# likojack/ODAM

Hardware: AMD Instinct MI355X
Metric: frames/sec end-to-end (DETR detect + SQ fit), 640x480 ScanNet, 1/2/4/8 GPU (higher is better)
Workload: dtype f32

## Files before the change

### include/odam_detr.h

```cpp
#ifndef ODAM_DETR_H
#define ODAM_DETR_H
#ifdef __cplusplus
extern "C" {
#endif

typedef struct odam_detr odam_detr;

typedef struct {
    int resnet_blocks[4];
    int hidden_dim;
    int nheads;
    int dim_feedforward;
    int enc_layers;
    int dec_layers;
    int num_queries;
    int num_classes1;
    int angle_bins;
    int max_batch;
    int img_h, img_w;
    int dtype;
    int pre_norm;
    int dilation;
    int basic_block;
} odam_detr_cfg;

int odam_detr_create(const odam_detr_cfg* cfg, odam_detr** out);
int odam_detr_destroy(odam_detr* m);

int odam_detr_set_weight(odam_detr* m, const char* name, const float* data, const long long* shape, int ndim);

int odam_detr_finalize(odam_detr* m);

int odam_detr_feature_hw(const odam_detr* m, int* h, int* w);

int odam_detr_forward(odam_detr* m, const float* img, int B, float* logits, float* boxes, float* angle,
                      float* offset, float* size, float* depth, float* obj_features, void* stream);

int odam_detr_forward_masked(odam_detr* m, const float* img, int B, const unsigned char* key_mask, const float* pos,
                             float* logits, float* boxes, float* angle, float* offset, float* size, float* depth,
                             float* obj_features, void* stream);

int odam_detr_forward_aux(odam_detr* m, const float* img, int B, const unsigned char* key_mask, const float* pos,
                          float* logits, float* boxes, float* angle, float* offset, float* size, float* depth,
                          float* obj_features, int frames_per_layer, void* stream);

int odam_detr_debug_read(odam_detr* m, int B, float* layer4_nchw, float* memory, void* stream);

int odam_detr_postprocess(odam_detr* m, const float* logits, const float* boxes, const float* angle,
                          const float* offset, const float* size, const float* depth, int B, const float* K9,
                          float img_w, float img_h, float* rows, void* stream);

int odam_detr_select(const float* rows, int Q, float threshold, int nms_2d, int* keep_idx, int* n_keep);

int odam_detr_select_pack(const float* rows16, int B, int Q, float threshold, int nms_2d, const float* frame_ids,
                          float seq_w, float seq_h, const float* sincos, int n_bins, float* det_block, int* det_count,
                          int* keep_idx, void* stream);

int odam_detr_preprocess_u8(odam_detr* m, const unsigned char* rgb, int B, int h, int w, const float* mean,
                            const float* std_dev, float* out, void* stream);

int odam_detr_profile_enable(odam_detr* m, int on);
int odam_detr_profile_read(odam_detr* m, int* n_launches, double* total_ms, double* total_flops);
int odam_detr_profile_read_attention(odam_detr* m, int* n_launches, double* total_ms, double* total_flops);


int odam_detr_profile_read_stages(odam_detr* m, int n, int* launches, double* ms, double* flops);

int odam_op_conv2d_nhwc(const float* x, const float* w_packed, const float* scale, const float* bias,
                        const float* residual, float* y, int B, int H, int W, int Cin, int Cout, int KH, int KW,
                        int stride, int pad, int Kpad, int relu, int k_order, void* stream);
int odam_op_conv2d_nhwc_bf16(const void* x, const void* w_packed, const float* scale, const float* bias,
                             const void* residual, void* y, int B, int H, int W, int Cin, int Cout, int KH, int KW,
                             int stride, int pad, int Kpad, int relu, int out_f32, int k_order, void* stream);
int odam_op_conv2d_nhwc_ex(const void* x, const void* w_packed, const float* scale, const float* bias, const void* residual,
                           void* y, int B, int H, int W, int Cin, int Cout, int KH, int KW, int stride, int pad, int dil,
                           int Kpad, int relu, int k_order, int dtype, int out_f32, void* stream);
int odam_op_bottleneck_bf16(const void* x, const void* w2, const float* s2, const float* b2, const void* w3, const float* s3,
                            const float* b3, const void* residual, void* y, const void* w1n, const float* s1n, const float* b1n,
                            void* y_next, int B, int H, int W, int P, int stride, int PN, void* stream);
int odam_op_bottleneck_f32(const float* x, const float* w2, const float* s2, const float* b2, const float* w3, const float* s3,
                           const float* b3, const float* residual, float* y, const float* w1n, const float* s1n, const float* b1n,
                           float* y_next, int B, int H, int W, int P, int stride, int PN, void* stream);
long long odam_op_conv_paths(char* buf, int n, int reset);
int odam_op_conv_bf16_mode(int mode);
int odam_op_conv_f32_mode(int mode);
long long odam_op_pooled_stem_launches(void);
int odam_op_attention(const float* Q, int ldq, const float* K, int ldk, const float* V, int ldv, float* O, int ldo,
                      int B, int H, int Lq, int Lk, void* stream);
int odam_op_attention_bf16(const void* Q, int ldq, const void* K, int ldk, const void* V, int ldv, void* O, int ldo,
                           int B, int H, int Lq, int Lk, void* stream);
int odam_op_add_layernorm(const float* x, const float* r, const float* gamma, const float* beta, float* y, int M,
                          void* stream);
int odam_op_attention_ex(const void* Q, int ldq, const void* K, int ldk, const void* V, int ldv, void* O, int ldo,
                         int B, int H, int Lq, int Lk, int head_dim, int dtype, const unsigned char* key_mask, void* stream);
int odam_op_add_layernorm_ex(const void* x, const void* r, const float* gamma, const float* beta, void* y,
                             const float* pos, int L, void* y_pos, int M, int dtype, void* stream);
int odam_op_attention_hd(const void* Q, int ldq, const void* K, int ldk, const void* V, int ldv, void* O, int ldo,
                         int B, int H, int Lq, int Lk, int head_dim, int dtype, const unsigned char* key_mask, void* stream);
int odam_op_add_layernorm_c(const void* x, const void* r, const float* gamma, const float* beta, void* y,
                            const float* pos, int L, void* y_pos, int M, int C, int dtype, void* stream);
int odam_op_quantize_mxfp8(const void* x, int src_dtype, long long n, void* q, void* s, void* stream);
int odam_op_dequantize_mxfp8(const void* q, const void* s, long long n, float* y, void* stream);
int odam_op_conv2d_nhwc_mxfp8(const void* x, const void* xs, const void* w_packed, const void* ws, const float* scale,
                              const float* bias, const void* residual, void* y, void* ys, void* y_bf16, float* y_f32,
                              int B, int H, int W, int Cin, int Cout, int KH, int KW, int stride, int pad, int dil,
                              int Kpad, int relu, int k_order, void* stream);
int odam_op_maxpool3x3s2_nhwc_ex(const void* x, void* y, int B, int H, int W, int C, int dtype, void* stream);
int odam_op_maxpool3x3s2_nhwc(const float* x, float* y, int B, int H, int W, int C, void* stream);
int odam_op_nchw_to_nhwc4(const float* in, void* out, int B, int H, int W, int dtype, int framed, void* stream);
int odam_op_nhwc_to_nchw(const void* in, float* out, int B, int H, int W, int C, int dtype, void* stream);
int odam_op_add_pos(const void* x, const float* pos, int L, void* out, int M, int C, int dtype, void* stream);
int odam_op_to_f32(const void* in, float* out, long long n, int dtype, void* stream);
int odam_op_sigmoid(float* x, int n, void* stream);
int odam_op_postprocess(const float* logits, const float* boxes, const float* angle, const float* offset, const float* size,
                        const float* depth, int n, int n_cls1, int n_bins, const float* K9, float img_w, float img_h, float* rows,
                        void* stream);

#ifdef __cplusplus
}
#endif
#endif
```

### odam_amd/_lib.py

```python
import ctypes
import os

_HERE = os.path.dirname(os.path.abspath(__file__))
LIB_PATH = os.environ.get("ODAM_AMD_LIB") or os.path.join(_HERE, "libodam_amd.so")
_lib = None

c_float_p = ctypes.POINTER(ctypes.c_float)
c_int_p = ctypes.POINTER(ctypes.c_int)
c_void_p = ctypes.c_void_p


class OdamError(RuntimeError):
    pass


_LEGACY_ENV = {"ODAM_CG_BIG": ("cg.ring", False), "ODAM_CG_BIG_F32": ("cg.f32", False), "ODAM_CG_FUSE": ("cg.fuse", False),
               "ODAM_CG_FUSE_BF16": ("cg.fuse_bf16", False), "ODAM_CG_S1": ("cg.s1", False), "ODAM_CG_NO_UT": ("cg.ut", True),
               "ODAM_CG_VARIANT": ("cg.tiles", False), "ODAM_CG_FORCE": ("cg.force", False), "ODAM_CG_NO_PRESPLIT": ("cg.presplit", True),
               "ODAM_ATT_X3": ("att.x3", False), "ODAM_ATT_FP32": ("att.bf16_mfma", True), "ODAM_STEM_ROWS": ("stem.rows", False),
               "ODAM_ASSOC_PERSIST": ("assoc.persist", False), "ODAM_SQ_SPLIT": ("sq.split", False),
               "ODAM_SQ_SPLIT_WAIT": ("sq.split_wait", False), "ODAM_SQ_S": ("sq.lanes", False)}


def _apply_env(L):
    pairs = []
    for name, (key, presence_means_off) in _LEGACY_ENV.items():
        if name in os.environ:
            pairs.append((key, 0 if presence_means_off else int(os.environ[name])))
    for item in filter(None, os.environ.get("ODAM_CONFIG", "").split(",")):
        k, v = item.split("=")
        pairs.append((k.strip(), int(v)))
    for k, v in pairs:
        if L.odam_config_set(k.encode(), ctypes.c_int(v)) != 0:
            raise OdamError(L.odam_last_error().decode("utf-8", "replace"))


def config():
    buf = ctypes.create_string_buffer(1024)
    check(lib().odam_config_describe(buf, 1024), "odam_config_describe")
    return {k: int(v.rstrip("*")) for k, v in (kv.split("=") for kv in buf.value.decode().split())}


def get_config(key):
    v = ctypes.c_int(0)
    check(lib().odam_config_get(key.encode(), ctypes.byref(v)), f"odam_config_get({key})")
    return v.value


def set_config(key, value):
    check(lib().odam_config_set(key.encode(), ctypes.c_int(int(value))), f"odam_config_set({key})")


_I, _P, _F = ctypes.c_int, ctypes.c_void_p, ctypes.c_float
_L, _D = ctypes.c_longlong, ctypes.c_double
_PROTOTYPES = {
    "odam_samples_create": [_I, _I, _L, _L, _P],
    "odam_samples_destroy": [_P],
    "odam_samples_load": [_P, _P, _P, _P, _P, _P, _P, _D, _D, _P],
    "odam_samples_cut": [_P, _I, _P, _P, _P, _I, _P, _P, _P, _P, _I, _P, _P, _P, _P],
    "odam_assoc_ot_batch": [_P, _P, _P, _P, _P, _I, _I, _F, _I, _P, _P, _P, _P, _P, _P, _P],
    "odam_assoc_reserve_batch": [_P, _I, _I],
    "odam_assoc_forward_batch": [_P, _P, _P, _P, _P, _I, _P, _P, _P, _P, _P, _P, _P],
}


def lib():
    global _lib
    if _lib is None:
        if not os.path.exists(LIB_PATH):
            raise OdamError(
                f"{LIB_PATH} not found: build it with `python -c 'import __graft_entry__ as g; g.build()'` "
                "(hipcc --offload-arch=gfx950). There is no CPU fallback.")
        import torch
        L = ctypes.CDLL(LIB_PATH)
        L.odam_last_error.restype = ctypes.c_char_p
        for name, argtypes in _PROTOTYPES.items():
            fn = getattr(L, name)
            fn.argtypes, fn.restype = argtypes, ctypes.c_int
        _apply_env(L)
        _lib = L
    return _lib


def check(code, what):
    if code != 0:
        msg = lib().odam_last_error().decode("utf-8", "replace")
        raise OdamError(f"{what} failed with code {code}: {msg}")


def ptr(t):
    if t is None:
        return c_void_p(0)
    return c_void_p(t.data_ptr())
```

### odam_amd/csrc/cg_args.h

```cpp
#pragma once

namespace odam_cg {

constexpr int ODAM_CG_F32 = 0;
constexpr int ODAM_CG_BF16 = 1;

struct ConvGemmArgs {
    const void* A;
    const void* Wt;
    const void* Wt3 = nullptr;
    const float* scale;
    const float* bias;
    const void* res;
    void* C;
    int B, H, W, Cin, log2Cin;
    int Ho, Wo, Cout;
    int KH, KW, stride, pad;
    int Kpad;
    int relu;
    int M;
    int ldc;
    int dtype;
    int out_f32;
    int lda;
    int k_order;
    const void* F_Wt3 = nullptr;
    const float* F_scale = nullptr;
    const float* F_bias = nullptr;
    const float* F_res = nullptr;
    float* F_C = nullptr;
    int F_ldc = 0, F_relu = 0;
    const void* G_Wt3 = nullptr;
    const float* G_scale = nullptr;
    const float* G_bias = nullptr;
    float* G_C = nullptr;
    int G_N = 64;
    const void* F_Wt = nullptr;
    const void* G_Wt = nullptr;
    int dil = 1;
    int pool = 0, pool_ph = 0, pool_pw = 0, Hp = 0, Wp = 0;
    int no_pin = 0;
    int s1_window = 0;
};

constexpr int POOL_PH = 8, POOL_PW = 14;

}
```

### odam_amd/csrc/cg_big.hpp

```cpp
#pragma once
#include "cg_common.hpp"
#include "cg_tails_f32.hpp"
#include "cg_tail_bf16.hpp"
#include "cg_launch.h"

namespace odam_cg {

constexpr int big_bm(int BN, int NTH) { return (NTH == 1024 && BN == 64) ? 512 : 256; }
constexpr int big_wm(int MODE, int BN, int NTH) {
    return NTH == 1024 ? (BN == 64 ? 16 : 4)
         : MODE >= 3 ? (BN == 256 ? ((MODE == 4 && CG_X16_WM8) ? 8 : 4) : 8) : (BN == 256 ? 2 : (BN == 128 ? 4 : 8));
}
#ifndef CG_DEEP_A
#define CG_DEEP_A 1
#endif

constexpr bool big_deep_a(int MODE, int BN, int NST, int NTH) { return CG_DEEP_A != 0 && MODE == 0 && BN == 256 && NST == 4 && NTH == 1024; }
template <int MODE, int BN, int NST, int NTH>
constexpr int big_lds_bytes() {
    const int bm = big_bm(BN, NTH);
    const int ring = NST * (MODE >= 3 ? bm * 64 + 96 * BN : (bm + BN) * 64);
    const int wm = big_wm(MODE, BN, NTH);
    const int wn = NTH / 64 / wm;
    const int slab = MODE == 4 ? (NTH / 64) * 16 * ((BN / wn > 128 ? 128 : BN / wn) + 4) * 4 : (NTH / 64) * 32 * (BN / wn) * 4;
    const int s1 = (MODE == 0 && NTH == 512) ? (BN == 256 ? 2 : (BN == 128 ? 3 : 4)) * (384 * 64 + 3 * BN * 64) : 0;
    const int m = ring > slab ? ring : slab;
    const int deep = big_deep_a(MODE, BN, NST, NTH) ? (6 + 4) * 256 * 64 : 0;
    const int m2 = m > s1 ? m : s1;
    return m2 > deep ? m2 : deep;
}

template <int MODE, int BN, int NST, int NTH = 512, int FUSE = 0>
__global__ __launch_bounds__(NTH, (NTH == 1024 ? 4 : 2)) void conv_gemm_big_kernel(ConvGemmArgs a) {
    static_assert(!FUSE || (FUSE <= 4 && (MODE == 3 || MODE == 4) && NTH == 512 && ((FUSE != 3 && BN == 64) || (FUSE == 3 && BN == 128))) ||
                      (FUSE >= 5 && FUSE <= 8 && MODE == 0 && NTH == 512 && NST == 4),
                  "fused layers: pre-split filters with 64-column tiles (FUSE 1, 2, 4) or 128-column tiles (FUSE 3); bf16 (FUSE 5 + "
                  "log2(PN / 32), 5 = no chained reduce)");
    static_assert(MODE == 0 || MODE == 2 || MODE == 3 || MODE == 4,
                  "bf16 operands, fp32 split, fp32 split with pre-split filters (3: 32x32x16 matrix instruction, 4: 16x16x32)");
    static_assert(MODE != 4 || FUSE <= 4, "the 16x16x32 schedule: its own epilogue, or the fp32 bottleneck tails");
    constexpr bool BF16 = MODE == 0;
    constexpr bool PRE = MODE == 3 || MODE == 4;
    constexpr bool X16 = MODE == 4;
    static_assert(!PRE || NTH == 512 || (X16 && NTH == 1024), "pre-split filters: eight-wave workgroups, or sixteen waves (16x16x32 loop)");
    static_assert(NTH != 1024 || (FUSE == 0 && ((BN == 64 && (X16 || BF16)) || (BN == 256 && BF16))), "sixteen waves: plain layers (512 x 64: bf16 or the 16x16x32 split loop; 256 x 256: bf16)");
    using T = typename std::conditional<BF16, unsigned short, float>::type;
    constexpr int EPC = BF16 ? 8 : 4;
    constexpr int BM = big_bm(BN, NTH), BKE = 4 * EPC;
    constexpr int KU = 2 * BKE;
    constexpr int NW = NTH / 64;
    constexpr int WM = big_wm(MODE, BN, NTH), WN = NW / WM;
    constexpr int TM = BM / WM / 32, TN = BN / WN / 32;
    constexpr int RPP = NTH / 4;
    constexpr int A_LD = BM / RPP, B_LD = (BN + RPP - 1) / RPP;
    constexpr int ROWB = 64;
    constexpr int A_BYTES = BM * ROWB;
    constexpr int STAGE = PRE ? A_BYTES + 3 * BN * 32 : (BM + BN) * ROWB;
    constexpr int NB3 = 3 * BN / 32;
    constexpr int B3_HI = (NB3 + NW - 1) / NW;
    constexpr int LPT = A_LD + (PRE ? B3_HI : B_LD);
    extern __shared__ __align__(16) float smem[];
    typedef __attribute__((address_space(3))) void* lds_ptr_t;
    const T* __restrict__ Ag = reinterpret_cast<const T*>(a.A);
    const T* __restrict__ Wg = reinterpret_cast<const T*>(a.Wt);

    const int tid = threadIdx.x, lane = tid & 63, wave = tid >> 6;
    const int wm = wave / WN, wn = wave % WN;
    const int tiles_n = (a.Cout + BN - 1) / BN;
    int bid = blockIdx.x;
#if CG_STAMP
    const unsigned long long st_entry = __builtin_readcyclecounter();
#endif
    {
        const int nwg = gridDim.x, xcd = bid & 7, q = nwg >> 3, r = nwg & 7;
        bid = (xcd < r ? xcd * (q + 1) : r * (q + 1) + (xcd - r) * q) + (bid >> 3);
    }
    const int tile_m = bid / tiles_n, tile_n = bid - tile_m * tiles_n;
    const int m0 = tile_m * BM, n0 = tile_n * BN;
    constexpr bool POOLABLE = NTH == 1024 && BN == 64 && FUSE == 0 && (MODE == 4 || MODE == 0);
    constexpr int pl_tw = 2 * POOL_PW + 1, pl_rows = (2 * POOL_PH + 1) * pl_tw;
    static_assert(pl_rows <= 512, "a patch fits a 512-row tile");
    int pl_b = 0, pl_y0 = 0, pl_x0 = 0;
    if constexpr (POOLABLE) {
        if (a.pool) {
            const int txs = (a.Wp + POOL_PW - 1) / POOL_PW, tys = (a.Hp + POOL_PH - 1) / POOL_PH;
            pl_b = bid / (tys * txs);
            const int rem = bid - pl_b * tys * txs, ty = rem / txs, tx = rem - ty * txs;
            pl_y0 = 2 * ty * POOL_PH - 1; pl_x0 = 2 * tx * POOL_PW - 1;
        }
    }
    auto pool_store = [&](const float* S) {
        constexpr int SLD = BN + 4;
        const int py0 = (pl_y0 + 1) >> 1, px0 = (pl_x0 + 1) >> 1;
        constexpr int items = POOL_PH * POOL_PW * (BN / 4);
        for (int it = tid; it < items; it += NTH) {
            const int c4p = it & (BN / 4 - 1), pp = it / (BN / 4), ppy = pp / POOL_PW, ppx = pp - ppy * POOL_PW;
            const int py = py0 + ppy, px = px0 + ppx;
            if (py >= a.Hp || px >= a.Wp) continue;
            const float* w0 = S + ((2 * ppy) * pl_tw + 2 * ppx) * SLD + c4p * 4;
            float4 m4 = *reinterpret_cast<const float4*>(w0);
#pragma unroll
            for (int dy = 0; dy < 3; dy++)
#pragma unroll
                for (int dx = 0; dx < 3; dx++) {
                    if (dy == 0 && dx == 0) continue;
                    const float4 v = *reinterpret_cast<const float4*>(w0 + (dy * pl_tw + dx) * SLD);
                    m4.x = fmaxf(m4.x, v.x); m4.y = fmaxf(m4.y, v.y); m4.z = fmaxf(m4.z, v.z); m4.w = fmaxf(m4.w, v.w);
                }
            const size_t o = (((size_t)pl_b * a.Hp + py) * a.Wp + px) * a.ldc + c4p * 4;
            if constexpr (BF16) {
                const unsigned lo = pack_bf16x2(m4.x, m4.y), hi = pack_bf16x2(m4.z, m4.w);
                *reinterpret_cast<uint2*>(reinterpret_cast<unsigned short*>(a.C) + o) = uint2{lo, hi};
            } else {
                *reinterpret_cast<float4*>(reinterpret_cast<float*>(a.C) + o) = m4;
            }
        }
    };
    auto pool_row_ok = [&](int R) {
        const int dy = R / pl_tw, oy = pl_y0 + dy, ox = pl_x0 + R - dy * pl_tw;
        return R < pl_rows && (unsigned)oy < (unsigned)a.Ho && (unsigned)ox < (unsigned)a.Wo;
    };

    const int c4 = tid & 3, r0 = tid >> 2;
    const int hw = a.Ho * a.Wo;
    const int lda = a.lda > 0 ? a.lda : a.Cin;
    const bool plain = a.KH * a.KW == 1 && a.stride == 1 && a.pad == 0;
    const int ntaps = a.KH * a.KW;
    const int kw_inv = (65536 + a.KW - 1) / a.KW;
    const int nt_inv = (65536 + ntaps - 1) / ntaps;
    const int b0 = (POOLABLE && a.pool) ? pl_b : m0 / hw;
    const int csrc = X16 ? (c4 ^ ((lane >> 4) & 1)) : (c4 ^ ((lane >> 4) & 3));
    const int margin = (a.pad * a.W + a.pad) * lda;
    const unsigned long long pa = (unsigned long long)(Ag + (size_t)b0 * a.H * a.W * lda - margin), pw = (unsigned long long)Wg;
    const u32x4 a_rs4 = u32x4{(unsigned)pa, (unsigned)(pa >> 32) & 0xffffu, OOB_VOFF, 0x00020000u};
    const u32x4 w_rs4 = u32x4{(unsigned)pw, (unsigned)(pw >> 32) & 0xffffu, OOB_VOFF, 0x00020000u};
    unsigned a_voff[A_LD], a_mask[A_LD], w_voff[B_LD];
#pragma unroll
    for (int i = 0; i < A_LD; i++) {
        const int m = m0 + r0 + RPP * i;
        bool ok = m < a.M;
        const int mm = ok ? m : 0;
        int base, iy0 = 0, ix0 = 0;
        if (POOLABLE && a.pool) {
            const int r = r0 + RPP * i, dy = r / pl_tw, oy = pl_y0 + dy, ox = pl_x0 + r - dy * pl_tw;
            ok = r < pl_rows && (unsigned)oy < (unsigned)a.Ho && (unsigned)ox < (unsigned)a.Wo;
            iy0 = (ok ? oy : 0) * a.stride - a.pad; ix0 = (ok ? ox : 0) * a.stride - a.pad;
            base = ((pl_b * a.H + iy0) * a.W + ix0) * lda;
        } else if (plain) {
            base = mm * lda;
        } else {
            const int b = mm / hw, rem = mm - b * hw, oy = rem / a.Wo, ox = rem - oy * a.Wo;
            iy0 = oy * a.stride - a.pad; ix0 = ox * a.stride - a.pad;
            base = ((b * a.H + iy0) * a.W + ix0) * lda;
        }
        a_voff[i] = (unsigned)(base - b0 * a.H * a.W * lda + margin + csrc * EPC) * (unsigned)sizeof(T);
        unsigned mk = plain ? 1u : 0u;
        for (int t = 0; t < (plain ? 0 : ntaps); t++) {
            const int ky = (t * kw_inv) >> 16, kx = t - ky * a.KW;
            if ((unsigned)(iy0 + ky * a.dil) < (unsigned)a.H && (unsigned)(ix0 + kx * a.dil) < (unsigned)a.W) mk |= 1u << t;
        }
        a_mask[i] = ok ? mk : 0u;
    }
#pragma unroll
    for (int i = 0; i < B_LD; i++) {
        const int n = n0 + r0 + RPP * i;
        w_voff[i] = (n < a.Cout && r0 + RPP * i < BN) ? (unsigned)(n * a.Kpad + csrc * EPC) * (unsigned)sizeof(T) : OOB_VOFF;
    }
    const unsigned lds_base = (unsigned)(size_t)(lds_ptr_t)smem;
    const int wave_u = __builtin_amdgcn_readfirstlane(wave);
    const bool b_wave = PRE ? (NB3 % NW == 0 || wave_u < NB3 % NW)
                            : (BN >= RPP || wave_u * 16 < BN);
    unsigned w3_voff[B3_HI > 0 ? B3_HI : 1];
    u32x4 w3_rs4 = w_rs4;
    if constexpr (PRE) {
        const unsigned long long p3 = (unsigned long long)a.Wt3;
        w3_rs4 = u32x4{(unsigned)p3, (unsigned)(p3 >> 32) & 0xffffu, OOB_VOFF, 0x00020000u};
#pragma unroll
        for (int j = 0; j < B3_HI; j++) {
            const int q = wave_u + NW * j;
            const int pl = q / (BN / 32), rb = q - pl * (BN / 32);
            const int row = rb * 32 + (lane >> 1);
            const int n = n0 + row;
            const int cs = X16 ? (lane & 1) : ((lane & 1) ^ ((lane >> 4) & 1));
            w3_voff[j] = (q < NB3 && n < a.Cout) ? (unsigned)(n * (a.Kpad / 16) * 96 + pl * 32 + cs * 16) : OOB_VOFF;
        }
    }

    struct TilePrep { int tap, soff_a, soff_b; };
    auto tile_prep = [&](int kt) {
        int tap, cbase;
        if (a.k_order) {
            const int ku = kt >> 1, chunk = (ku * nt_inv) >> 16;
            tap = ku - chunk * ntaps;
            cbase = chunk * KU + (kt & 1) * BKE;
        } else {
            const int kb = kt * BKE;
            tap = kb >> a.log2Cin;
            cbase = kb & (a.Cin - 1);
        }
        const int ky = (tap * kw_inv) >> 16, kx = tap - ky * a.KW;
        return TilePrep{tap, ((ky * a.W + kx) * a.dil * lda + cbase) * (int)sizeof(T), PRE ? kt * 96 : kt * BKE * (int)sizeof(T)};
    };
    auto dma_part = [&](const TilePrep& tp, int st, int part) {
        const unsigned sb = lds_base + (unsigned)(st * STAGE + wave_u * 16 * ROWB);
        if (part < A_LD) {
            const unsigned vo = ((a_mask[part] >> tp.tap) & 1u) ? a_voff[part] : OOB_VOFF;
            lds_dma16(a_rs4, sb + (unsigned)(RPP * part * ROWB), vo, tp.soff_a);
        } else if constexpr (PRE) {
// ... 86 lines not shown
            for (int j = 0; j < TN; j++) {
                b0[j] = *reinterpret_cast<const float4*>(Bb + j * 32 * ROWB + fq[0]);
                b1[j] = *reinterpret_cast<const float4*>(Bb + j * 32 * ROWB + fq[1]);
            }
            a0 = *reinterpret_cast<const float4*>(Ab + fq[0]);
            a1 = *reinterpret_cast<const float4*>(Ab + fq[1]);
            int part = 0;
            issue_next(part++);
#pragma unroll
            for (; part < LPT; part++) issue_next(part);
#pragma unroll
            for (int j = 0; j < TN; j++) split8(b0[j], b1[j], bh[j], bm[j], bl[j]);
#pragma unroll
            for (int i = 0; i < TM; i++) {
                uint4 ah, am, al;
                split8(a0, a1, ah, am, al);
                if (i + 1 < TM) {
                    a0 = *reinterpret_cast<const float4*>(Ab + (i + 1) * 32 * ROWB + fq[0]);
                    a1 = *reinterpret_cast<const float4*>(Ab + (i + 1) * 32 * ROWB + fq[1]);
                }
#define ODAM_MM(x, y) acc[i][j] = __builtin_amdgcn_mfma_f32_32x32x16_bf16(__builtin_bit_cast(bf16x8, x), __builtin_bit_cast(bf16x8, y), acc[i][j], 0, 0, 0)
#pragma unroll
                for (int j = 0; j < TN; j++) {
                    ODAM_MM(al, bh[j]); ODAM_MM(am, bm[j]); ODAM_MM(ah, bl[j]);
                    ODAM_MM(am, bh[j]); ODAM_MM(ah, bm[j]);
                    ODAM_MM(ah, bh[j]);
                }
#undef ODAM_MM
            }
            return;
        }
        mma_ab(Ab, Bb, issue_next);
    };

    const int nk = a.Kpad / BKE;
    if constexpr (X16) {
        constexpr int MI = BM / WM / 16, NJ = BN / WN / 16;
        static_assert(NJ % 4 == 0, "column tiles in groups of four");
        floatx4 c16[MI][NJ];
#pragma unroll
        for (int i = 0; i < MI; i++)
#pragma unroll
            for (int j = 0; j < NJ; j++) c16[i][j] = floatx4{0.f, 0.f, 0.f, 0.f};
        const int r16 = lane & 15, kq = lane >> 4;
        const int akey = (r16 >> 2) & 1;
        const int a_lane = (kq >> 1) * STAGE + (wm * (BM / WM) + r16) * ROWB;
        const int a_c0 = ((2 * (kq & 1)) ^ akey) << 4, a_c1 = ((2 * (kq & 1) + 1) ^ akey) << 4;
        const int b_lane = (kq >> 1) * STAGE + A_BYTES + (wn * (BN / WN) + r16) * 32 + (kq & 1) * 16;
        auto dma_tile = [&](int kt, int st) {
            if (kt >= nk) return;
            const TilePrep tp = tile_prep(kt);
#pragma unroll
            for (int part = 0; part < A_LD; part++) {
                const unsigned vo = ((a_mask[part] >> tp.tap) & 1u) ? a_voff[part] : OOB_VOFF;
                lds_dma16(a_rs4, lds_base + (unsigned)(st * STAGE + wave_u * 16 * ROWB + RPP * part * ROWB), vo, tp.soff_a);
            }
#pragma unroll
            for (int j = 0; j < B3_HI; j++)
                if (j + 1 < B3_HI || b_wave)
                    lds_dma16(w3_rs4, lds_base + (unsigned)(st * STAGE + A_BYTES + (wave_u + NW * j) * 1024), w3_voff[j], tp.soff_b);
        };
        constexpr int NBLK = MI * NJ;
        constexpr int NDMA = 2 * (A_LD + B3_HI);
        auto dma_part16 = [&](int kt, int st, int part) {
            if (kt >= nk) return;
            const TilePrep tp = tile_prep(kt);
            if (part < A_LD) {
                const unsigned vo = ((a_mask[part] >> tp.tap) & 1u) ? a_voff[part] : OOB_VOFF;
                lds_dma16(a_rs4, lds_base + (unsigned)(st * STAGE + wave_u * 16 * ROWB + RPP * part * ROWB), vo, tp.soff_a);
            } else {
                const int j = part - A_LD;
                if (j + 1 < B3_HI || b_wave)
                    lds_dma16(w3_rs4, lds_base + (unsigned)(st * STAGE + A_BYTES + (wave_u + NW * j) * 1024), w3_voff[j < B3_HI ? j : 0], tp.soff_b);
            }
        };
        dma_tile(0, 0); dma_tile(1, 1);
#if CG_HACK & 3
        const size_t hk_off = ((size_t)m0 * a.ldc + n0) * sizeof(float);
        const __amdgpu_buffer_rsrc_t hk_res = __builtin_amdgcn_make_buffer_rsrc(const_cast<char*>(reinterpret_cast<const char*>(a.res ? a.res : a.C)) + hk_off, 0, a.res ? (int)OOB_VOFF : 0, 0x00020000);
        const __amdgpu_buffer_rsrc_t hk_out = __builtin_amdgcn_make_buffer_rsrc(reinterpret_cast<char*>(a.C) + hk_off, 0, (int)OOB_VOFF, 0x00020000);
        u32x4 hk_l[8] = {};
        constexpr int HK_LPR = (BN / WN) / 4, HK_RPI = 64 / HK_LPR;
        const int hk_row0 = wm * (BM / WM) + lane / HK_LPR;
        const unsigned hk_col = (unsigned)(wn * (BN / WN) + (lane % HK_LPR) * 4) * 4u;
#endif
#define ODAM_MM16(accv, x, y) accv = __builtin_amdgcn_mfma_f32_16x16x32_bf16(__builtin_bit_cast(bf16x8, x), __builtin_bit_cast(bf16x8, y), accv, 0, 0, 0)
#if CG_STAMP
        unsigned long long st_acc[4] = {0, 0, 0, 0}, st_prev = __builtin_readcyclecounter();
        const unsigned long long st_loop0 = st_prev;
#endif
        for (int kp = 0; 2 * kp < nk; ++kp) {
            CG_STAMP_AT(3);
            asm volatile("s_waitcnt vmcnt(0)" ::: "memory");
            CG_STAMP_AT(1);
            __builtin_amdgcn_s_barrier();
            asm volatile("" ::: "memory");
            CG_STAMP_AT(0);
            const int s0 = (2 * kp) & 3;
            const char* Sa = lds_c + s0 * STAGE + a_lane;
            const char* Sb = lds_c + s0 * STAGE + b_lane;
            struct Ops { uint4 h, m, l; };
            constexpr int BD = 2;
            Ops A2[2], B2[BD + 1];
            float4 ar0, ar1;
            auto read_b = [&](int nj, Ops& o) {
                const char* bp = Sb + nj * 16 * 32;
                o.h = *reinterpret_cast<const uint4*>(bp);
                o.m = *reinterpret_cast<const uint4*>(bp + BN * 32);
                o.l = *reinterpret_cast<const uint4*>(bp + 2 * BN * 32);
            };
            auto read_a = [&](int mi) {
                ar0 = *reinterpret_cast<const float4*>(Sa + mi * 16 * ROWB + a_c0);
                ar1 = *reinterpret_cast<const float4*>(Sa + mi * 16 * ROWB + a_c1);
            };
            auto half_split = [](const float4& c, Ops& o, int hf) {
                const float v[4] = {c.x, c.y, c.z, c.w};
                unsigned uh[4], um[4], ul[4];
#pragma unroll
                for (int e = 0; e < 4; e++) {
                    uh[e] = __builtin_bit_cast(unsigned, v[e]);
                    const float r1 = v[e] - __builtin_bit_cast(float, uh[e] & 0xffff0000u);
                    um[e] = __builtin_bit_cast(unsigned, r1);
                    ul[e] = __builtin_bit_cast(unsigned, r1 - __builtin_bit_cast(float, um[e] & 0xffff0000u));
                }
                auto pk = [](unsigned lo_, unsigned hi_) { return __builtin_amdgcn_perm(hi_, lo_, 0x07060302u); };
                if (hf == 0) {
                    o.h.x = pk(uh[0], uh[1]); o.h.y = pk(uh[2], uh[3]); o.m.x = pk(um[0], um[1]); o.m.y = pk(um[2], um[3]);
                    o.l.x = pk(ul[0], ul[1]); o.l.y = pk(ul[2], ul[3]);
                } else {
                    o.h.z = pk(uh[0], uh[1]); o.h.w = pk(uh[2], uh[3]); o.m.z = pk(um[0], um[1]); o.m.w = pk(um[2], um[3]);
                    o.l.z = pk(ul[0], ul[1]); o.l.w = pk(ul[2], ul[3]);
                }
            };
            constexpr bool BREG = CG_X16_BREG != 0;
            constexpr int NG = NJ / 4;
            Ops A4[BREG ? MI : 1], Bg[BREG ? 4 : 1];
            read_a(0);
            if constexpr (BREG) {
#pragma unroll
                for (int j = 0; j < 4; j++) read_b(j, Bg[j]);
                half_split(ar0, A4[0], 0); half_split(ar1, A4[0], 1);
            } else {
#pragma unroll
// ... 532 lines not shown
        return;
    }
    if constexpr (FUSE == 4) {
        fused_chain128(a, acc, smem, lds_base, m0, wave, lane);
        return;
    }
    if constexpr (POOLABLE && MODE == 0) {
        if (a.pool) {
            constexpr int SLD = BN + 4;
            static_assert(BM * SLD * 4 <= big_lds_bytes<MODE, BN, NST, NTH>(), "the pooling slab fits the ring");
            float* S = smem;
            const int half = lane >> 5, l32 = lane & 31;
#pragma unroll
            for (int i = 0; i < TM; i++)
#pragma unroll
                for (int j = 0; j < TN; j++) {
                    const int n = wn * (BN / WN) + j * 32 + l32;
                    const float sc = a.scale ? a.scale[n] : 1.0f, bi = a.bias ? a.bias[n] : 0.0f;
#pragma unroll
                    for (int r = 0; r < 16; r++) {
                        const int R = wm * (BM / WM) + i * 32 + (r & 3) + 8 * (r >> 2) + 4 * half;
                        float v = acc[i][j][r] * sc + bi;
                        v = bf2f(f2bf(v));
                        S[R * SLD + n] = (pool_row_ok(R) && v > 0.f) ? v : 0.f;
                    }
                }
            __syncthreads();
            pool_store(S);
            return;
        }
    }
    if constexpr (FUSE >= 5) {
        fused_bf16<BN, FUSE == 5 ? 0 : (32 << (FUSE - 5)), FUSE == 7 ? 2 : 3>(a, acc, smem, lds_base, m0, wm, wn, wave, lane);
        return;
    }
    static_assert(X16 || (WM * WN * 32 * (BN / WN) * 4 <= big_lds_bytes<MODE, BN, NST, NTH>() && NST * STAGE <= big_lds_bytes<MODE, BN, NST, NTH>()),
                  "ring and epilogue staging fit the dynamic LDS");
    if (ep2) epilogue2<BM, BN, WM, WN, TM, TN, BF16>(a, acc, smem, m0, n0, wm, wn, wave, lane);
    else epilogue<BM, BN, WM, WN, TM, TN, BF16>(a, acc, smem, big_lds_bytes<MODE, BN, NST, NTH>() / 4, m0, n0, wm, wn, wave, lane);
}

template <int MODE, int BN, int NST, int NTH = 512>
static int launch_big(const ConvGemmArgs& a_in, int s1_window, hipStream_t stream) {
    ConvGemmArgs a = a_in;
    a.s1_window = s1_window;
    constexpr int bytes = big_lds_bytes<MODE, BN, NST, NTH>();
    static const bool attr_ok = [] {
        return hipFuncSetAttribute((const void*)conv_gemm_big_kernel<MODE, BN, NST, NTH>, hipFuncAttributeMaxDynamicSharedMemorySize, bytes) == hipSuccess;
    }();
    if (!attr_ok) return odam_fail(2, "conv_gemm: cannot raise the dynamic LDS limit");
    constexpr int bm = big_bm(BN, NTH);
    int tiles = ((a.M + bm - 1) / bm) * ((a.Cout + BN - 1) / BN);
    if (a.pool) {
        if (!(NTH == 1024 && BN == 64 && (MODE == 4 || MODE == 0)) || a.Cout != 64 || a.pool_ph != POOL_PH || a.pool_pw != POOL_PW ||
            a.ldc != a.Cout || a.res)
            return odam_fail(1, "conv_gemm: pooled stem asked for where it does not apply");
        tiles = a.B * ((a.Hp + POOL_PH - 1) / POOL_PH) * ((a.Wp + POOL_PW - 1) / POOL_PW);
    }
    hipLaunchKernelGGL((conv_gemm_big_kernel<MODE, BN, NST, NTH>), dim3(tiles), dim3(NTH), bytes, stream, a);
    ODAM_HIP(hipGetLastError());
    return 0;
}


}
```

### odam_amd/csrc/cg_big_f32.hip

```cpp
#include "cg_big.hpp"

namespace odam_cg {

int launch_big_f32(int mode, int bn, int nth, const ConvGemmArgs& a, hipStream_t stream) {
    if (nth == 1024) {
        if (mode == 4 && bn == 64) return launch_big<4, 64, 4, 1024>(a, 0, stream);
    } else if (bn == 256) {
        if (mode == 4) return launch_big<4, 256, 4>(a, 0, stream);
        if (mode == 3) return launch_big<3, 256, 4>(a, 0, stream);
        if (mode == 2) return launch_big<2, 256, 4>(a, 0, stream);
    } else if (bn == 128) {
        if (mode == 4) return launch_big<4, 128, 4>(a, 0, stream);
        if (mode == 3) return launch_big<3, 128, 4>(a, 0, stream);
        if (mode == 2) return launch_big<2, 128, 4>(a, 0, stream);
    } else if (bn == 64) {
        if (mode == 4) return launch_big<4, 64, 4>(a, 0, stream);
        if (mode == 3) return launch_big<3, 64, 4>(a, 0, stream);
        if (mode == 2) return launch_big<2, 64, 4>(a, 0, stream);
    }
    return odam_fail(1, "conv_gemm: ring kernel (fp32): tile shape not built");
}

}
```

### odam_amd/csrc/cg_choice.h

```cpp
#pragma once
#include "cg_args.h"

namespace odam_cg {

struct Switches {
    int ring, f32, fuse, fuse_bf16, s1, ut, tiles, force, presplit, mfma16, pin, small_x3, stem_pool;
};
Switches current_switches();

enum class Family { Refused, Nothing, Small, RingF32, RingBF16, FusedF32, FusedBF16 };

struct Choice {
    Family family = Family::Nothing;
    bool bf16 = false;
    int bm = 0, bn = 0, waves = 0;
    int stages = 2;
    bool ut = false, x3 = false;
    int mode = 0;
    bool pool = false;
    int chain = 0;
    int s1_window = 0;
    int code = 0;
    const char* message = nullptr;
};

Choice choose(const ConvGemmArgs& a, const Switches& sw);

constexpr int PATH_TOKEN_LEN = 40;
void choice_token(const Choice& c, char* tok);

bool fused_second_ok(const ConvGemmArgs& a, const Switches& sw);
bool fused_bf16_ok(const ConvGemmArgs& a, const Switches& sw);
bool pooled_stem_ok(const ConvGemmArgs& a, const Switches& sw);
bool fused_second_ok(const ConvGemmArgs& a);
bool fused_bf16_ok(const ConvGemmArgs& a);
bool pooled_stem_ok(const ConvGemmArgs& a);
bool presplit_applies(int Cout, int Kpad);

void set_big_mode(int mode);
void set_f32_mode(int mode);
int f32_mode();

}
```

### odam_amd/csrc/cg_choice.hip

```cpp
#include "cg_choice.h"

#include <cstdio>

#include "odam_config.h"

namespace odam_cg {

Switches current_switches() {
    using namespace odam_cfg;
    return {get(CG_RING), get(CG_F32),      get(CG_FUSE),   get(CG_FUSE_BF16), get(CG_S1),       get(CG_UT),    get(CG_TILES),
            get(CG_FORCE), get(CG_PRESPLIT), get(CG_MFMA16), get(CG_PIN),       get(CG_SMALL_X3), get(STEM_POOL)};
}

void set_big_mode(int mode) { odam_cfg::set(odam_cfg::CG_RING, mode); }
void set_f32_mode(int mode) { odam_cfg::set(odam_cfg::CG_F32, mode == 1 ? 0 : mode); }
int f32_mode() {
    const Switches sw = current_switches();
    return sw.ring ? sw.f32 : 0;
}

namespace {

inline bool is_bf16(const ConvGemmArgs& a) { return a.dtype == ODAM_CG_BF16; }

// ... 49 lines not shown
    return c;
}

Choice small_tiles(const ConvGemmArgs& a, const Switches& sw, int bm, int bn, int waves, bool deep = false) {
    Choice c;
    c.family = Family::Small;
    c.bf16 = is_bf16(a);
    c.bm = bm; c.bn = bn; c.waves = waves;
    c.ut = sw.ut != 0 && a.Cin % (c.bf16 ? 64 : 32) == 0 && a.KH * a.KW <= 32 && offsets_fit(a, bm);
    c.x3 = !c.bf16 && c.ut && sw.f32 == 2 && sw.small_x3 != 0;
    c.stages = (c.ut && deep) ? 4 : 2;
    return c;
}

}

bool fused_second_ok(const ConvGemmArgs& a, const Switches& sw) {
    if (!sw.fuse || !sw.ring || sw.f32 != 2 || a.dtype != ODAM_CG_F32) return false;
    if (!a.F_Wt3 || !a.F_C || !a.Wt3) return false;
    const bool l1 = a.Cout == 64 && a.F_ldc == 256, l2 = a.Cout == 128 && a.F_ldc == 512 && !a.G_Wt3;
    if ((!l1 && !l2) || a.dil != 1) return false;
    if (!split_planes_fit(a.Cout, a.Kpad) || !fits31((long)a.Ho * a.Wo * a.F_ldc * 4)) return false;
    if (a.G_Wt3 && (sw.fuse < 2 || !a.G_C || (a.G_N != 64 && a.G_N != 128))) return false;
    return ring_eligible(a, sw, a.Cout);
}

bool fused_bf16_ok(const ConvGemmArgs& a, const Switches& sw) {
    if (!sw.fuse_bf16 || !sw.ring || a.dtype != ODAM_CG_BF16 || !a.F_Wt || !a.F_C) return false;
    if (a.Cout != 64 && a.Cout != 128 && a.Cout != 256) return false;
    if (a.F_ldc != 4 * a.Cout || a.KH * a.KW != 9 || a.Cin != a.Cout || !a.k_order || a.dil != 1) return false;
    if (!fits31((long)a.M * a.F_ldc * 2)) return false;
    if (a.G_Wt) {
        if (sw.fuse_bf16 < 2 || !a.G_C) return false;
        const bool built = (a.Cout == 64 && (a.G_N == 64 || a.G_N == 128)) || (a.Cout == 128 && a.G_N == 128);
        if (!built) return false;
    }
    return ring_eligible(a, sw, a.Cout);
}

bool pooled_stem_ok(const ConvGemmArgs& a, const Switches& sw) {
    if (!sw.ring || !(sw.tiles & 8) || sw.stem_pool == 0) return false;
    if (is_bf16(a)) {
        if (!(a.lda > 0 && a.lda < a.Cin) && sw.ring < 2) return false;
        if (is_3x3_stride1(a) || a.out_f32) return false;
    } else if (ring_mode_f32(a, sw) != 4) {
        return false;
    }
    if (a.Cout != 64 || a.ldc != 64 || a.res || !a.relu) return false;
    if (a.pool_ph != POOL_PH || a.pool_pw != POOL_PW) return false;
    if (a.Hp != (a.Ho + 2 - 3) / 2 + 1 || a.Wp != (a.Wo + 2 - 3) / 2 + 1) return false;
    return ring_eligible(a, sw, 64) && fills_512_row_tiles(a, sw);
}

bool fused_second_ok(const ConvGemmArgs& a) { return fused_second_ok(a, current_switches()); }
bool fused_bf16_ok(const ConvGemmArgs& a) { return fused_bf16_ok(a, current_switches()); }
bool pooled_stem_ok(const ConvGemmArgs& a) { return pooled_stem_ok(a, current_switches()); }
bool presplit_applies(int Cout, int Kpad) { return f32_mode() == 2 && split_planes_fit(Cout, Kpad); }

Choice choose(const ConvGemmArgs& a, const Switches& sw) {
    const bool bf = is_bf16(a);
    const int epc = bf ? 8 : 4, taps = a.KH * a.KW;
    if (a.Kpad % (8 * epc) != 0 || a.Cin < epc || (a.Cin & (a.Cin - 1)) != 0 || a.KW > 7 || taps > 64)
        return refuse("conv_gemm: unsupported shape (Kpad % k-tile, Cin a power of two >= one 16-byte chunk, KW <= 7)");
    if (a.k_order && (a.Cin % (8 * epc) != 0 || taps > 32 || a.Kpad / (8 * epc) >= 2048))
        return refuse("conv_gemm: k_order 1 needs Cin % k-tile == 0, at most 32 taps, fewer than 2048 k-tiles");
    if (a.M <= 0 || a.Cout <= 0) return Choice{};

    if (a.pool) {
        if (!pooled_stem_ok(a, sw)) return refuse("conv_gemm: pooled stem asked for where it does not apply (check pooled_stem_ok)");
        return ring(a, sw, bf ? 0 : 4, 64, 16);
    }
    if (a.F_Wt3) {
        if (!fused_second_ok(a, sw)) return refuse("conv_gemm: fused second layer asked for where it does not apply (check fused_second_ok)");
        Choice c;
        c.family = Family::FusedF32;
        c.bm = 256; c.bn = a.Cout; c.waves = 8; c.chain = a.G_Wt3 ? a.G_N : 0;
        c.mode = (a.Kpad % 32 == 0 && (sw.mfma16 >= 3 || (sw.mfma16 == 2 && a.Cout == 128))) ? 4 : 3;
        return c;
    }
    if (a.F_Wt) {
        if (!fused_bf16_ok(a, sw)) return refuse("conv_gemm: fused bf16 bottleneck asked for where it does not apply (check fused_bf16_ok)");
        Choice c;
        c.family = Family::FusedBF16;
        c.bf16 = true;
        c.bm = 256; c.bn = a.Cout; c.waves = 8; c.chain = a.G_Wt ? a.G_N : 0;
        c.s1_window = sw.s1;
        return c;
    }

    if (sw.ring) {
        const bool x3 = !bf && sw.f32 == 2;
        const int mode = bf ? 0 : ring_mode_f32(a, sw);
        if (a.Cout % 256 == 0 || a.Cout >= 384) {
            if (ring_eligible(a, sw, 256))
                return ring(a, sw, mode, 256, (bf && (sw.tiles & 16) && !is_3x3_stride1(a)) ? 16 : 8);
            if (mode >= 3 && ring_eligible(a, sw, 128)) return ring(a, sw, mode, 128, 8);
        } else if (a.Cout > 64 && (sw.ring >= 2 || x3) && ring_eligible(a, sw, 128)) {
            return ring(a, sw, mode, 128, 8);
        } else if (x3 && a.Cout > 32 && a.Cout <= 64 && ring_eligible(a, sw, 64)) {
            return ring(a, sw, mode, 64, (mode == 4 && (sw.tiles & 8) && fills_512_row_tiles(a, sw)) ? 16 : 8);
        } else if (bf && (sw.ring >= 2 || (a.lda > 0 && a.lda < a.Cin)) && a.Cout > 32 && a.Cout <= 64 && ring_eligible(a, sw, 64)) {
            return ring(a, sw, mode, 64, ((sw.tiles & 8) && !is_3x3_stride1(a) && fills_512_row_tiles(a, sw)) ? 16 : 8);
        }
    }

    if (sw.force == 1) return small_tiles(a, sw, 128, 64, 8);
    if (sw.force == 2) return small_tiles(a, sw, 64, 64, 4, true);
    if (sw.force == 3) return small_tiles(a, sw, 128, 128, 4);
    if (a.Cout <= 64) return small_tiles(a, sw, 128, 64, (sw.tiles & 2) ? 8 : 4);
    const long tiles128 = (long)((a.M + 127) / 128) * ((a.Cout + 127) / 128);
    if (tiles128 < 128) return small_tiles(a, sw, 64, 64, 4, (sw.tiles & 4) != 0);
    return small_tiles(a, sw, 128, 128, (sw.tiles & 1) ? 8 : 4);
}

void choice_token(const Choice& c, char* tok) {
    const int n = PATH_TOKEN_LEN;
    tok[0] = 0;
    switch (c.family) {
    case Family::Small:
        std::snprintf(tok, n, "%s.small.%dx%d.w%d%s%s%s", c.bf16 ? "bf16" : "f32", c.bm, c.bn, c.waves, c.ut ? ".ut" : "", c.x3 ? ".x3" : "",
// ... 18 lines not shown
```

### odam_amd/csrc/detr_forward.hip

```cpp
#include <hip/hip_runtime.h>

#include <atomic>

#include "detr_kernels.h"
#include "detr_model.h"
#include "odam_config.h"

using namespace odam_dm;
using odam_cg::ConvGemmArgs;

namespace odam_dm {

ConvGemmArgs conv_args(const Conv& c, const void* x, int B, int H, int W, int dtype) {
    ConvGemmArgs a{};
    a.dtype = dtype;
    a.A = x; a.Wt = c.w; a.Wt3 = c.w3; a.scale = c.scale; a.bias = c.bias;
    a.B = B; a.H = H; a.W = W; a.Cin = c.Cin; a.log2Cin = ilog2(c.Cin);
    a.Ho = conv_out(H, (c.KH - 1) * c.dil + 1, c.stride, c.pad); a.Wo = conv_out(W, (c.KW - 1) * c.dil + 1, c.stride, c.pad);
    a.Cout = c.Cout; a.KH = c.KH; a.KW = c.KW; a.stride = c.stride; a.pad = c.pad; a.Kpad = c.Kpad; a.dil = c.dil;
    a.k_order = c.k_order;
    a.M = B * a.Ho * a.Wo; a.ldc = c.Cout;
    return a;
}

// ... 27 lines not shown
    const int Ho = conv_out(H, (c.KH - 1) * c.dil + 1, c.stride, c.pad), Wo = conv_out(W, (c.KW - 1) * c.dil + 1, c.stride, c.pad);
    const int Cin_true = (c.KH == 7) ? 3 : c.Cin;
    return m->conv_ev.timed(st, 2.0 * B * Ho * Wo * (double)c.Cout * c.KH * c.KW * Cin_true,
                            [&] { return run_conv(c, x, B, H, W, res, relu, y, st, m->dt, out_f32); });
}
int lin_t(odam_detr* m, const Conv& c, const void* x, int M, const void* res, bool relu, void* y, hipStream_t st,
          int out_f32 = 0) {
    return conv_t(m, c, x, 1, 1, M, res, relu, y, st, out_f32);
}

int fused_c2c3_t(odam_detr* m, const Conv& c2, const Conv& c3, const void* x, int B, int H, int W, const void* res, void* y,
                 hipStream_t st, const Conv* next_c1, void* t_next, bool* chained) {
    *chained = false;
    if (m->basic) return -1;
    if (c2.dil != 1) return -1;
    if (c3.KH != 1 || c3.stride != 1 || c3.Kpad != c2.Cout) return -1;
    if (!m->dt && (!c2.w3 || !c3.w3)) return -1;
    ConvGemmArgs a = conv_args(c2, x, B, H, W, m->dt);
    a.relu = 1;
    a.F_scale = c3.scale; a.F_bias = c3.bias; a.F_res = (const float*)res; a.F_C = (float*)y;
    a.F_ldc = c3.Cout; a.F_relu = 1;
    const bool bf = m->dt != 0;
    auto fused_ok = [&] { return bf ? odam_cg::fused_bf16_ok(a) : odam_cg::fused_second_ok(a); };
    if (bf) a.F_Wt = c3.w; else a.F_Wt3 = c3.w3;
    const bool next_ok = next_c1 && t_next && next_c1->KH == 1 && next_c1->stride == 1 && next_c1->Kpad == c3.Cout &&
                         (bf || (next_c1->w3 && (next_c1->Cout == 64 || next_c1->Cout == 128) && c3.Cout == 256));
    if (next_ok) {
        if (bf) a.G_Wt = next_c1->w; else a.G_Wt3 = next_c1->w3;
        a.G_scale = next_c1->scale; a.G_bias = next_c1->bias; a.G_C = (float*)t_next; a.G_N = next_c1->Cout;
        *chained = fused_ok();
        if (!*chained) { a.G_Wt = a.G_Wt3 = nullptr; a.G_scale = a.G_bias = nullptr; a.G_C = nullptr; a.G_N = 64; }
    }
    if (!fused_ok()) return -1;
    const double flops3 = *chained ? 2.0 * a.M * (double)next_c1->Cout * c3.Cout : 0.0;
    return m->conv_ev.timed(st, 2.0 * a.M * ((double)c2.Cout * c2.KH * c2.KW * c2.Cin + (double)c3.Cout * c2.Cout) + flops3,
                            [&] { return odam_cg::launch_conv_gemm(a, st); });
}

std::atomic<long long> g_pooled_stem_launches{0};

int stem_rows_t(odam_detr* m, int B, hipStream_t st, void* pooled_out, bool* pooled) {
    const Conv& c = m->stem_rows;
    ConvGemmArgs a = conv_args(c, m->x4, B, m->cfg.img_h + 6, m->cfg.img_w + 8, m->dt);
    a.lda = 4; a.Ho = m->H1; a.Wo = m->W1; a.M = B * a.Ho * a.Wo;
    a.relu = 1;
    a.pool = 1; a.pool_ph = odam_cg::POOL_PH; a.pool_pw = odam_cg::POOL_PW; a.Hp = m->H2; a.Wp = m->W2; a.C = pooled_out;
    *pooled = odam_cg::pooled_stem_ok(a);
    if (!*pooled) { a.pool = 0; a.C = m->stem_out; }
    else g_pooled_stem_launches.fetch_add(1);
    return m->conv_ev.timed(st, 2.0 * a.M * (double)c.Cout * 147,
                            [&] { return odam_cg::launch_conv_gemm(a, st); });
}

int mx_t(odam_detr* m, const Conv& c, const unsigned char* x, const unsigned char* xs, int B, int H, int W, const void* res, bool relu,
         unsigned char* y, unsigned char* ys, void* yb, hipStream_t st) {
    odam_mx::ConvArgs a = mx_args(c, x, xs, B, H, W);
    a.res = (const unsigned short*)res; a.relu = relu ? 1 : 0;
    a.y = y; a.ys = ys; a.yb = (unsigned short*)yb;
    return m->conv_ev.timed(st, 2.0 * a.M * (double)c.Cout * c.Kpad, [&] { return odam_mx::launch_conv(a, st); });
}

int att_t(odam_detr* m, const void* Q, int ldq, const void* K, int ldk, const void* V, int ldv, void* O, int ldo,
          int B, int H, int Lq, int Lk, hipStream_t st, const unsigned char* key_mask = nullptr) {
    const int hd = m->cfg.hidden_dim / m->cfg.nheads;
    return m->att_ev.timed(st, 4.0 * B * H * (double)Lq * Lk * hd,
                           [&] { return odam_dk::launch_attention(Q, ldq, K, ldk, V, ldv, O, ldo, B, H, Lq, Lk, m->dt, st, key_mask, hd); });
}


struct Act { char *cur, *nxt; int H, W; };

char* off(const odam_detr* m, char* p, size_t n) { return p + n * m->es; }

void mark_stage(odam_detr* m, size_t i) {
    for (int l = 0, first = 0; l < 4; first += m->cfg.resnet_blocks[l], l++)
        if ((int)i == first) m->stage_ev[l + 1] = m->conv_ev.used;
}

int stem(odam_detr* m, const float* img, int B, hipStream_t st) {
    const int dt = m->dt, ih = m->cfg.img_h, iw = m->cfg.img_w;
    const bool rows_ok = odam_cfg::get(odam_cfg::STEM_ROWS) != 0;
    bool pooled = false;
    const long Mst = (long)B * m->H1 * m->W1;
    const bool rows_mode = dt ? (m->stem_rows.w != nullptr && odam_cfg::get(odam_cfg::CG_RING) != 0)
                              : (m->stem_rows.w3 != nullptr && odam_cg::f32_mode() == 2);
    if (rows_ok && rows_mode && (Mst >= 192L * 256 || odam_cfg::get(odam_cfg::CG_PIN))) {
        RC(odam_dk::launch_nchw_to_nhwc4_framed(img, m->x4, B, ih, iw, dt, st));
        RC(stem_rows_t(m, B, st, m->bufA, &pooled));
    } else {
        RC(odam_dk::launch_nchw_to_nhwc4(img, m->x4, B, ih, iw, dt, st));
        RC(conv_t(m, m->stem, m->x4, B, ih, iw, nullptr, true, m->stem_out, st));
    }
    if (!pooled) RC(odam_dk::launch_maxpool3x3s2(m->stem_out, m->bufA, B, m->H1, m->W1, 64, m->H2, m->W2, dt, st));
    return 0;
}

int body_mxfp8(odam_detr* m, int B, Act& s, hipStream_t st) {
    unsigned char *cq = m->qa, *cs = m->qas, *nq = m->qb, *ns = m->qbs;
    RC(odam_mx::launch_quantize(s.cur, 1, (size_t)B * s.H * s.W * 64, cq, cs, st));
    for (size_t i = 0; i < m->blocks.size(); i++) {
        mark_stage(m, i);
        const Bottleneck& b = m->blocks[i];
        const int stride = m->block_stride[i];
        const int Ho = conv_out(s.H, 3, stride, 1), Wo = conv_out(s.W, 3, stride, 1);
        const bool last = i + 1 == m->blocks.size();
        unsigned char* oq = last ? nullptr : nq;
        unsigned char* os = last ? nullptr : ns;
        RC(mx_t(m, b.c1, cq, cs, B, s.H, s.W, nullptr, true, m->qt1, m->qt1s, nullptr, st));
        const char* res = s.cur;
        if (b.has_ds) {
            RC(mx_t(m, b.ds, cq, cs, B, s.H, s.W, nullptr, false, nullptr, nullptr, m->dsb, st));
            res = m->dsb;
        }
        if (m->basic) {
            RC(mx_t(m, b.c2, m->qt1, m->qt1s, B, Ho, Wo, res, true, oq, os, s.nxt, st));
        } else {
            RC(mx_t(m, b.c2, m->qt1, m->qt1s, B, s.H, s.W, nullptr, true, m->qt2, m->qt2s, nullptr, st));
            RC(mx_t(m, b.c3, m->qt2, m->qt2s, B, Ho, Wo, res, true, oq, os, s.nxt, st));
        }
        std::swap(s.cur, s.nxt); std::swap(cq, nq); std::swap(cs, ns);
        s.H = Ho; s.W = Wo;
    }
    return 0;
}

int body_basic(odam_detr* m, int B, Act& s, hipStream_t st) {
    for (size_t i = 0; i < m->blocks.size(); i++) {
        mark_stage(m, i);
        const Bottleneck& b = m->blocks[i];
        const int stride = m->block_stride[i];
        const int Ho = conv_out(s.H, 3, stride, 1), Wo = conv_out(s.W, 3, stride, 1);
        RC(conv_t(m, b.c1, s.cur, B, s.H, s.W, nullptr, true, m->t1, st));
        const char* res = s.cur;
        if (b.has_ds) {
            RC(conv_t(m, b.ds, s.cur, B, s.H, s.W, nullptr, false, m->dsb, st));
            res = m->dsb;
        }
        RC(conv_t(m, b.c2, m->t1, B, Ho, Wo, res, true, s.nxt, st));
        std::swap(s.cur, s.nxt);
        s.H = Ho; s.W = Wo;
    }
    return 0;
}

int body_bottleneck(odam_detr* m, int B, Act& s, hipStream_t st) {
    char* tin = m->t1;
    char* tout = m->t2;
    bool have_c1 = false;
// ... 71 lines not shown
        RC(lin_t(m, m->mlp[k][2], m->h2, Mq, nullptr, false, outs[k], st, 1));
    }
    return odam_dk::launch_sigmoid(boxes, Mq * 4, st);
}

struct LayerOut { float *logits, *boxes, *angle, *offset, *size, *depth, *obj_features; int fpl; };

int layer_heads(odam_detr* m, int B, const LayerOut& o, size_t l, hipStream_t st) {
    const size_t row = l * (size_t)o.fpl * m->cfg.num_queries;
    return heads(m, B, o.logits + row * m->cfg.num_classes1, o.boxes + row * 4, o.angle + row * m->cfg.angle_bins, o.offset + row * 2,
                 o.size + row * 3, o.depth + row, o.obj_features ? o.obj_features + row * m->cfg.hidden_dim : nullptr, st);
}

int decoder(odam_detr* m, int B, const unsigned char* key_mask, hipStream_t st, const LayerOut* each = nullptr) {
    const int E = m->cfg.hidden_dim, Hh = m->cfg.nheads, Q = m->cfg.num_queries, dt = m->dt, L = m->L, Mq = B * Q;
    ODAM_HIP(hipMemsetAsync(m->tgt, 0, (size_t)m->es * Mq * E, st));
    RC(odam_dk::launch_add_pos(nullptr, m->query_pos, Q, m->tgtpos, Mq, dt, st, E));
    const int ldkv = m->cfg.dec_layers * E;
    for (size_t i = 0; i < m->dec.size(); i++) {
        const DecLayer& d = m->dec[i];
        if (m->cfg.pre_norm) {
            RC(odam_dk::launch_add_layernorm(m->tgt, nullptr, d.n1.g, d.n1.b, m->dtmp, m->query_pos, Q, m->tgtpos, Mq, dt, st, E));
            RC(lin_t(m, d.qk, m->tgtpos, Mq, nullptr, false, m->dqk, st));
            RC(lin_t(m, d.v, m->dtmp, Mq, nullptr, false, m->dv, st));
            RC(att_t(m, m->dqk, 2 * E, off(m, m->dqk, E), 2 * E, m->dv, E, m->datt, E, B, Hh, Q, Q, st));
            RC(lin_t(m, d.out, m->datt, Mq, m->tgt, false, m->tgt, st));
            RC(odam_dk::launch_add_layernorm(m->tgt, nullptr, d.n2.g, d.n2.b, m->dtmp, m->query_pos, Q, m->tgtpos, Mq, dt, st, E));
            RC(lin_t(m, d.cq, m->tgtpos, Mq, nullptr, false, m->dq, st));
            RC(att_t(m, m->dq, E, off(m, m->kc, i * E), ldkv, off(m, m->vc, i * E), ldkv, m->datt, E, B, Hh, Q, L, st, key_mask));
            RC(lin_t(m, d.cout, m->datt, Mq, m->tgt, false, m->tgt, st));
            RC(odam_dk::launch_add_layernorm(m->tgt, nullptr, d.n3.g, d.n3.b, m->dtmp, nullptr, Q, nullptr, Mq, dt, st, E));
            RC(lin_t(m, d.l1, m->dtmp, Mq, nullptr, true, m->dffn, st));
            RC(lin_t(m, d.l2, m->dffn, Mq, m->tgt, false, m->tgt, st));
            if (each) RC(layer_heads(m, B, *each, i, st));
            continue;
        }
        RC(lin_t(m, d.qk, m->tgtpos, Mq, nullptr, false, m->dqk, st));
        RC(lin_t(m, d.v, m->tgt, Mq, nullptr, false, m->dv, st));
        RC(att_t(m, m->dqk, 2 * E, off(m, m->dqk, E), 2 * E, m->dv, E, m->datt, E, B, Hh, Q, Q, st));
        RC(lin_t(m, d.out, m->datt, Mq, m->tgt, false, m->dtmp, st));
        RC(odam_dk::launch_add_layernorm(m->dtmp, nullptr, d.n1.g, d.n1.b, m->tgt, m->query_pos, Q, m->tgtpos, Mq, dt, st, E));
        RC(lin_t(m, d.cq, m->tgtpos, Mq, nullptr, false, m->dq, st));
        RC(att_t(m, m->dq, E, off(m, m->kc, i * E), ldkv, off(m, m->vc, i * E), ldkv, m->datt, E, B, Hh, Q, L, st, key_mask));
        RC(lin_t(m, d.cout, m->datt, Mq, m->tgt, false, m->dtmp, st));
        RC(odam_dk::launch_add_layernorm(m->dtmp, nullptr, d.n2.g, d.n2.b, m->tgt, nullptr, Q, nullptr, Mq, dt, st, E));
        RC(lin_t(m, d.l1, m->tgt, Mq, nullptr, true, m->dffn, st));
        RC(lin_t(m, d.l2, m->dffn, Mq, m->tgt, false, m->dtmp, st));
        RC(odam_dk::launch_add_layernorm(m->dtmp, nullptr, d.n3.g, d.n3.b, m->tgt, m->query_pos, Q, m->tgtpos, Mq, dt, st, E));
        if (each) RC(layer_heads(m, B, *each, i, st));
    }
    return 0;
}

int forward_impl(odam_detr* m, const float* img, int B, const unsigned char* key_mask, const float* pos_b,
                 float* logits, float* boxes, float* angle, float* offset, float* size, float* depth,
                 float* obj_features, void* stream, int frames_per_layer = 0) {
    if (!m || !img || !logits || !boxes || !angle || !offset || !size || !depth)
        return odam_fail(1, "odam_detr_forward: null pointer");
    if (!m->finalized) return odam_fail(1, "odam_detr_forward: call odam_detr_finalize first");
    if (B < 1 || B > m->cfg.max_batch) return odam_fail(3, "odam_detr_forward: batch outside 1..max_batch");
    hipStream_t st = (hipStream_t)stream;
    m->conv_ev.used = m->att_ev.used = 0;

    RC(stem(m, img, B, st));
    std::fill(m->stage_ev, m->stage_ev + 6, m->conv_ev.used);
    m->stage_ev[0] = 0;
    Act s{m->bufA, m->bufB, m->H2, m->W2};
    RC(m->mx ? body_mxfp8(m, B, s, st) : m->basic ? body_basic(m, B, s, st) : body_bottleneck(m, B, s, st));
    m->layer4 = s.cur;
    m->stage_ev[5] = m->conv_ev.used;

    const int E = m->cfg.hidden_dim, M = B * m->L;
    RC(conv_t(m, m->input_proj, s.cur, B, s.H, s.W, nullptr, false, m->src, st));
    const float* pos = pos_b ? pos_b : m->pos;
    const int Lp = pos_b ? M : m->L;
    RC(odam_dk::launch_add_pos(m->src, pos, Lp, m->srcpos, M, m->dt, st, E));
    RC(encoder(m, B, pos, Lp, key_mask, st));
    RC(lin_t(m, m->cross_k_all, m->srcpos, M, nullptr, false, m->kc, st));
    RC(lin_t(m, m->cross_v_all, m->memory_out, M, nullptr, false, m->vc, st));

    if (frames_per_layer > 0) {
        const LayerOut each{logits, boxes, angle, offset, size, depth, obj_features, frames_per_layer};
        return decoder(m, B, key_mask, st, &each);
    }
    RC(decoder(m, B, key_mask, st));
    return heads(m, B, logits, boxes, angle, offset, size, depth, obj_features, st);
}

}

extern "C" int odam_detr_forward(odam_detr* m, const float* img, int B, float* logits, float* boxes, float* angle,
                                 float* offset, float* size, float* depth, float* obj_features, void* stream) {
    return forward_impl(m, img, B, nullptr, nullptr, logits, boxes, angle, offset, size, depth, obj_features, stream);
}

extern "C" int odam_detr_forward_masked(odam_detr* m, const float* img, int B, const unsigned char* key_mask,
                                        const float* pos, float* logits, float* boxes, float* angle, float* offset,
                                        float* size, float* depth, float* obj_features, void* stream) {
    if (!key_mask || !pos) return odam_fail(1, "odam_detr_forward_masked: null mask / position table");
    return forward_impl(m, img, B, key_mask, pos, logits, boxes, angle, offset, size, depth, obj_features, stream);
}

extern "C" int odam_detr_forward_aux(odam_detr* m, const float* img, int B, const unsigned char* key_mask, const float* pos,
                                     float* logits, float* boxes, float* angle, float* offset, float* size, float* depth,
                                     float* obj_features, int frames_per_layer, void* stream) {
    if (!m || !img || !logits || !boxes || !angle || !offset || !size || !depth) return odam_fail(1, "odam_detr_forward_aux: null pointer");
    if ((key_mask == nullptr) != (pos == nullptr))
        return odam_fail(1, "odam_detr_forward_aux: mask and position table go together (both null for a same-size batch)");
    if (frames_per_layer < 1 || frames_per_layer < B) return odam_fail(1, "odam_detr_forward_aux: frames_per_layer below the batch");
    if (!m->finalized) return odam_fail(1, "odam_detr_forward_aux: call odam_detr_finalize first");
    return forward_impl(m, img, B, key_mask, pos, logits, boxes, angle, offset, size, depth, obj_features, stream, frames_per_layer);
}

extern "C" int odam_detr_debug_read(odam_detr* m, int B, float* layer4_nchw, float* memory, void* stream) {
    if (!m || !m->finalized || !m->layer4) return odam_fail(1, "odam_detr_debug_read: no forward has run");
    hipStream_t st = (hipStream_t)stream;
    if (layer4_nchw) RC(odam_dk::launch_nhwc_to_nchw(m->layer4, layer4_nchw, B, m->fh, m->fw, m->l4_ch, m->dt, st));
    if (memory) RC(odam_dk::launch_to_f32(m->memory_out ? m->memory_out : m->src, memory, (size_t)B * m->L * m->cfg.hidden_dim, m->dt, st));
    return 0;
}

extern "C" int odam_detr_postprocess(odam_detr* m, const float* logits, const float* boxes, const float* angle,
                                     const float* offset, const float* size, const float* depth, int B,
                                     const float* K9, float img_w, float img_h, float* rows, void* stream) {
    if (!m || !logits || !boxes || !angle || !offset || !size || !depth || !K9 || !rows)
        return odam_fail(1, "odam_detr_postprocess: null pointer");
    return odam_dk::launch_postprocess(logits, boxes, angle, offset, size, depth, B, m->cfg.num_queries,
                                       m->cfg.num_classes1, m->cfg.angle_bins, img_w, img_h, K9[0], K9[4], K9[2],
                                       K9[5], rows, (hipStream_t)stream);
}

extern "C" long long odam_op_pooled_stem_launches(void) { return g_pooled_stem_launches.load(); }

extern "C" int odam_detr_profile_enable(odam_detr* m, int on) {
    if (!m) return odam_fail(1, "odam_detr_profile_enable: null model");
    m->conv_ev.on = m->att_ev.on = on != 0;
    m->conv_ev.used = m->att_ev.used = 0;
    return 0;
}

extern "C" int odam_detr_profile_read(odam_detr* m, int* n_launches, double* total_ms, double* total_flops) {
    if (!m || !n_launches || !total_ms || !total_flops) return odam_fail(1, "odam_detr_profile_read: null argument");
    return m->conv_ev.sum(0, m->conv_ev.used, n_launches, total_ms, total_flops);
}

extern "C" int odam_detr_profile_read_stages(odam_detr* m, int n, int* launches, double* ms, double* flops) {
// ... 11 lines not shown
```

### odam_amd/csrc/detr_input.hip

```cpp
#include <hip/hip_runtime.h>

#include <cmath>

#include "detr_kernels.h"
#include "detr_model.h"

using namespace odam_dm;

static int resample_table(odam_detr* m, int in_size, int out_size, odam_detr::Resample* r) {
    auto it = m->resample.find({in_size, out_size});
    if (it != m->resample.end()) { *r = it->second; return 0; }
    const double scale = (double)in_size / out_size;
    const double filterscale = scale < 1.0 ? 1.0 : scale;
    const double support = 1.0 * filterscale;
    const int ksize = (int)std::ceil(support) * 2 + 1;
    std::vector<int> xmin(out_size), cnt(out_size), K((size_t)out_size * ksize, 0);
    std::vector<double> w(ksize);
    const double ss = 1.0 / filterscale;
    for (int xx = 0; xx < out_size; xx++) {
        const double center = (xx + 0.5) * scale;
        int lo = (int)(center - support + 0.5);
        if (lo < 0) lo = 0;
        int hi = (int)(center + support + 0.5);
        if (hi > in_size) hi = in_size;
        const int n = hi - lo;
        double ww = 0.0;
        for (int x = 0; x < ksize; x++) w[x] = 0.0;
        for (int x = 0; x < n; x++) {
            double t = (x + lo - center + 0.5) * ss;
            if (t < 0.0) t = -t;
            w[x] = t < 1.0 ? 1.0 - t : 0.0;
            ww += w[x];
        }
        for (int x = 0; x < n; x++)
            if (ww != 0.0) w[x] /= ww;
        for (int x = 0; x < ksize; x++)
            K[(size_t)xx * ksize + x] = w[x] < 0 ? (int)(-0.5 + w[x] * (1 << 22)) : (int)(0.5 + w[x] * (1 << 22));
        xmin[xx] = lo; cnt[xx] = n;
    }
    odam_detr::Resample t{};
    t.ksize = ksize;
    if (int rc = m->dev_alloc(&t.xmin, xmin.size())) return rc;
    if (int rc = m->dev_alloc(&t.cnt, cnt.size())) return rc;
    if (int rc = m->dev_alloc(&t.K, K.size())) return rc;
    ODAM_HIP(hipMemcpy(t.xmin, xmin.data(), xmin.size() * sizeof(int), hipMemcpyHostToDevice));
    ODAM_HIP(hipMemcpy(t.cnt, cnt.data(), cnt.size() * sizeof(int), hipMemcpyHostToDevice));
    ODAM_HIP(hipMemcpy(t.K, K.data(), K.size() * sizeof(int), hipMemcpyHostToDevice));
    m->resample[{in_size, out_size}] = t;
    *r = t;
    return 0;
}

extern "C" int odam_detr_preprocess_u8(odam_detr* m, const unsigned char* rgb, int B, int h, int w, const float* mean,
                                       const float* stdv, float* out, void* stream) {
    if (!m || !rgb || !mean || !stdv || !out) return odam_fail(1, "odam_detr_preprocess_u8: null pointer");
    if (B < 0 || h < 1 || w < 1) return odam_fail(1, "odam_detr_preprocess_u8: bad size");
    odam_detr::Resample tx{}, ty{};
    RC(resample_table(m, w, m->cfg.img_w, &tx));
    RC(resample_table(m, h, m->cfg.img_h, &ty));
    return odam_dk::launch_preprocess_u8(rgb, B, h, w, tx.xmin, tx.cnt, tx.K, tx.ksize, ty.xmin, ty.cnt, ty.K, ty.ksize,
                                         out, m->cfg.img_h, m->cfg.img_w, mean, stdv, (hipStream_t)stream);
}

extern "C" int odam_detr_select(const float* rows, int Q, float threshold, int nms_2d, int* keep_idx, int* n_keep) {
    if (!rows || !keep_idx || !n_keep || Q < 0) return odam_fail(1, "odam_detr_select: bad argument");
    std::vector<int> cand;
    for (int q = 0; q < Q; q++)
        if (rows[(size_t)q * 16] > threshold) cand.push_back(q);
    std::stable_sort(cand.begin(), cand.end(), [&](int a, int b) { return rows[(size_t)a * 16] < rows[(size_t)b * 16]; });
    std::reverse(cand.begin(), cand.end());
    const int n = (int)cand.size();
    std::vector<char> sup(n, 0);
    auto box3 = [&](int q, float lo[3], float hi[3]) {
        const float* r = rows + (size_t)q * 16;
        for (int k = 0; k < 3; k++) {
            lo[k] = (-r[10 + k]) / 2.0f + r[6 + k];
            hi[k] = r[10 + k] / 2.0f + r[6 + k];
        }
    };
    int nk = 0;
    for (int i = 0; i < n; i++) {
        if (sup[i]) continue;
        const int s = cand[i];
        keep_idx[nk++] = s;
        float slo[3], shi[3];
        box3(s, slo, shi);
        const float* rs = rows + (size_t)s * 16;
        for (int j = i + 1; j < n; j++) {
            if (sup[j]) continue;
            const int t = cand[j];
            const float* rt = rows + (size_t)t * 16;
            float tlo[3], thi[3];
            box3(t, tlo, thi);
            float inter = 1.0f, va = 1.0f, vb = 1.0f;
            {
                const float dx = std::max(0.0f, std::min(shi[0], thi[0]) - std::max(slo[0], tlo[0]));
                const float dy = std::max(0.0f, std::min(shi[1], thi[1]) - std::max(slo[1], tlo[1]));
                const float dz = std::max(0.0f, std::min(shi[2], thi[2]) - std::max(slo[2], tlo[2]));
                inter = dx * dy * dz;
                va = (shi[0] - slo[0]) * (shi[1] - slo[1]) * (shi[2] - slo[2]);
                vb = (thi[0] - tlo[0]) * (thi[1] - tlo[1]) * (thi[2] - tlo[2]);
            }
            const float iou3 = inter / (va + vb - inter);
// ... 15 lines not shown
```

### odam_amd/csrc/detr_kernels.h

```cpp
#pragma once
#include <hip/hip_runtime.h>

namespace odam_dk {

int launch_attention(const void* Q, int ldq, const void* K, int ldk, const void* V, int ldv, void* O, int ldo,
                     int B, int H, int Lq, int Lk, int dtype, hipStream_t stream, const unsigned char* key_mask = nullptr,
                     int head_dim = 32);

int launch_attention_d64(const float* Q, int ldq, const float* K, int ldk, const float* V, int ldv, float* O, int ldo,
                         int B, int H, int Lq, int Lk, hipStream_t stream);

int launch_add_layernorm(const void* x, const void* r, const float* gamma, const float* beta, void* y,
                         const float* pos, int L, void* y_pos, int M, int dtype, hipStream_t stream, int C = 256);

int launch_add_pos(const void* x, const float* pos, int L, void* out, int M, int dtype, hipStream_t stream, int C = 256);

int launch_nchw_to_nhwc4(const float* in, void* out, int B, int H, int W, int dtype, hipStream_t stream);
int launch_nchw_to_nhwc4_framed(const float* in, void* out, int B, int H, int W, int dtype, hipStream_t stream);

int launch_maxpool3x3s2(const void* in, void* out, int B, int H, int W, int C, int Ho, int Wo, int dtype,
                        hipStream_t stream);

int launch_nhwc_to_nchw(const void* in, float* out, int B, int H, int W, int C, int dtype, hipStream_t stream);

int launch_to_f32(const void* in, float* out, size_t n, int dtype, hipStream_t stream);

int launch_sigmoid(float* x, int n, hipStream_t stream);

int launch_postprocess(const float* logits, const float* boxes, const float* angle, const float* offset,
                       const float* size, const float* depth, int B, int Q, int n_cls1, int n_bins, float img_w,
                       float img_h, float fx, float fy, float cx, float cy, float* rows, hipStream_t stream);

int launch_preprocess_u8(const unsigned char* rgb, int B, int h, int w, const int* tx_xmin, const int* tx_cnt,
                         const int* tx_K, int tx_ksize, const int* ty_xmin, const int* ty_cnt, const int* ty_K,
                         int ty_ksize, float* out, int H, int W, const float mean[3], const float stdv[3],
                         hipStream_t stream);

}
```

### odam_amd/csrc/detr_kernels.hip

```cpp
#include "detr_kernels.h"

#include <cstdlib>

#include "odam_config.h"
#include "odam_err.h"

namespace odam_dk {

typedef float floatx16 __attribute__((ext_vector_type(16)));
typedef unsigned short bf16_t;

__device__ __forceinline__ float bf2f(bf16_t u) { return __builtin_bit_cast(float, (unsigned)u << 16); }
__device__ __forceinline__ bf16_t f2bf(float f) { return __builtin_bit_cast(bf16_t, (__bf16)f); }
__device__ __forceinline__ unsigned pack_bf16x2(float lo, float hi) {
    typedef float f32x2_t __attribute__((ext_vector_type(2)));
    typedef __bf16 bf16x2_t __attribute__((ext_vector_type(2)));
    return __builtin_bit_cast(unsigned, __builtin_convertvector(f32x2_t{lo, hi}, bf16x2_t));
}
__device__ __forceinline__ float4 ld4(const float* p) { return *reinterpret_cast<const float4*>(p); }
__device__ __forceinline__ float4 ld4(const bf16_t* p) {
    const ushort4 u = *reinterpret_cast<const ushort4*>(p);
    return float4{bf2f(u.x), bf2f(u.y), bf2f(u.z), bf2f(u.w)};
}
__device__ __forceinline__ void st4(float* p, float4 v) { *reinterpret_cast<float4*>(p) = v; }
__device__ __forceinline__ void st4(bf16_t* p, float4 v) {
    *reinterpret_cast<uint2*>(p) = uint2{pack_bf16x2(v.x, v.y), pack_bf16x2(v.z, v.w)};
}
#define ODAM_DISPATCH(dtype, KERNEL, ...)                                                  \
    do {                                                                                  \
        if ((dtype) == 1) { KERNEL(bf16_t, __VA_ARGS__); } else { KERNEL(float, __VA_ARGS__); } \
    } while (0)

constexpr int ATT_KT = 32;

__device__ __forceinline__ int acc_row(int r, int half) { return (r & 3) + 8 * (r >> 2) + 4 * half; }

template <typename T, int D>
__global__ __launch_bounds__(256) void attention_kernel(const T* __restrict__ Q, int ldq,
                                                        const T* __restrict__ K, int ldk,
                                                        const T* __restrict__ V, int ldv,
                                                        T* __restrict__ O, int ldo, int Lq, int Lk, float scale,
                                                        const unsigned char* __restrict__ key_mask) {
    constexpr int LD = D + 4;
    constexpr int HD = D / 2;
    constexpr int NO = D / 32;
    constexpr int CPR = D / 4;
    constexpr int RPP = 256 / CPR;
    __shared__ __align__(16) float Ks[2][ATT_KT][LD];
    __shared__ __align__(16) float Vs[2][ATT_KT][LD];

    const int tid = threadIdx.x, lane = tid & 63, wave = tid >> 6;
    const int half = lane >> 5, col = lane & 31;
    const int h = blockIdx.y, b = blockIdx.z;
    const int q0 = blockIdx.x * 128 + wave * 32;
    const T* Qb = Q + (size_t)b * Lq * ldq + h * D;
    const T* Kb = K + (size_t)b * Lk * ldk + h * D;
    const T* Vb = V + (size_t)b * Lk * ldv + h * D;

// ... 827 lines not shown
    float den = 0.0f;
    for (int c = 0; c < n_cls1; c++) den += expf(lg[c] - mx);
    float best = -1.0f;
    int cls = 0;
    for (int c = 0; c < n_cls1 - 1; c++) {
        const float p = expf(lg[c] - mx) / den;
        if (p > best) { best = p; cls = c; }
    }
    const float* bx = boxes + (size_t)i * 4;
    const float x0 = (bx[0] - 0.5f * bx[2]) * img_w, y0 = (bx[1] - 0.5f * bx[3]) * img_h;
    const float x1 = (bx[0] + 0.5f * bx[2]) * img_w, y1 = (bx[1] + 0.5f * bx[3]) * img_h;
    const float d = depth[i];
    const float scx = offset[(size_t)i * 2 + 0] * img_w + (x0 + x1) / 2.0f;
    const float scy = offset[(size_t)i * 2 + 1] * img_h + (y0 + y1) / 2.0f;
    const float c3x = ((scx - cx) / fx) * d;
    const float c3y = ((scy - cy) / fy) * d;
    const float* an = angle + (size_t)i * n_bins;
    int ab = 0;
    float am = an[0];
    for (int k = 1; k < n_bins; k++)
        if (an[k] > am) { am = an[k]; ab = k; }
    float* o = rows + (size_t)i * 16;
    o[0] = best; o[1] = (float)cls;
    o[2] = x0; o[3] = y0; o[4] = x1; o[5] = y1;
    o[6] = c3x; o[7] = c3y; o[8] = d;
    o[9] = (float)ab;
    o[10] = size[(size_t)i * 3 + 0]; o[11] = size[(size_t)i * 3 + 1]; o[12] = size[(size_t)i * 3 + 2];
    o[13] = 0.0f; o[14] = 0.0f; o[15] = 0.0f;
}

int launch_postprocess(const float* logits, const float* boxes, const float* angle, const float* offset,
                       const float* size, const float* depth, int B, int Q, int n_cls1, int n_bins, float img_w,
                       float img_h, float fx, float fy, float cx, float cy, float* rows, hipStream_t stream) {
    const int n = B * Q;
    if (n <= 0) return 0;
    hipLaunchKernelGGL(postprocess_kernel, dim3((n + 63) / 64), dim3(64), 0, stream, logits, boxes, angle, offset,
                       size, depth, n, n_cls1, n_bins, img_w, img_h, fx, fy, cx, cy, rows);
    ODAM_HIP(hipGetLastError());
    return 0;
}

struct ResampleTable {
    const int* xmin;
    const int* cnt;
    const int* K;
    int ksize;
};

__device__ __forceinline__ int clip8_22(int v) {
    v >>= 22;
    return v < 0 ? 0 : (v > 255 ? 255 : v);
}

__global__ __launch_bounds__(256) void preprocess_u8_kernel(const unsigned char* __restrict__ rgb, int h, int w,
                                                            ResampleTable tx, ResampleTable ty, int need_x, int need_y,
                                                            float* __restrict__ out, int H, int W, float3 mean,
                                                            float3 stdv) {
    const int X = blockIdx.x * 256 + threadIdx.x;
    const int Y = blockIdx.y;
    const size_t b = blockIdx.z;
    if (X >= W) return;
    const unsigned char* img = rgb + b * (size_t)h * w * 3;
    const int x0 = need_x ? tx.xmin[X] : X, nx = need_x ? tx.cnt[X] : 1;
    const int y0 = need_y ? ty.xmin[Y] : Y, ny = need_y ? ty.cnt[Y] : 1;
    const int* kx = tx.K + (size_t)X * tx.ksize;
    const int* ky = ty.K + (size_t)Y * ty.ksize;
    int acc[3] = {1 << 21, 1 << 21, 1 << 21};
    int last[3] = {0, 0, 0};
    for (int j = 0; j < ny; j++) {
        const unsigned char* row = img + ((size_t)(y0 + j) * w + x0) * 3;
        int hv[3];
        if (need_x) {
            int a0 = 1 << 21, a1 = 1 << 21, a2 = 1 << 21;
            for (int k = 0; k < nx; k++) {
                const int kk = kx[k];
                a0 += row[k * 3 + 0] * kk; a1 += row[k * 3 + 1] * kk; a2 += row[k * 3 + 2] * kk;
            }
            hv[0] = clip8_22(a0); hv[1] = clip8_22(a1); hv[2] = clip8_22(a2);
        } else {
            hv[0] = row[0]; hv[1] = row[1]; hv[2] = row[2];
        }
        if (need_y) {
            const int kk = ky[j];
            acc[0] += hv[0] * kk; acc[1] += hv[1] * kk; acc[2] += hv[2] * kk;
        }
        last[0] = hv[0]; last[1] = hv[1]; last[2] = hv[2];
    }
    const int u0 = need_y ? clip8_22(acc[0]) : last[0];
    const int u1 = need_y ? clip8_22(acc[1]) : last[1];
    const int u2 = need_y ? clip8_22(acc[2]) : last[2];
    const size_t plane = (size_t)H * W, o = (b * 3 * H + Y) * (size_t)W + X;
    out[o] = ((float)u0 / 255.0f - mean.x) / stdv.x;
    out[o + plane] = ((float)u1 / 255.0f - mean.y) / stdv.y;
    out[o + 2 * plane] = ((float)u2 / 255.0f - mean.z) / stdv.z;
}

int launch_preprocess_u8(const unsigned char* rgb, int B, int h, int w, const int* tx_xmin, const int* tx_cnt,
                         const int* tx_K, int tx_ksize, const int* ty_xmin, const int* ty_cnt, const int* ty_K,
                         int ty_ksize, float* out, int H, int W, const float mean[3], const float stdv[3],
                         hipStream_t stream) {
    if (B <= 0) return 0;
    ResampleTable tx{tx_xmin, tx_cnt, tx_K, tx_ksize}, ty{ty_xmin, ty_cnt, ty_K, ty_ksize};
    hipLaunchKernelGGL(preprocess_u8_kernel, dim3((W + 255) / 256, H, B), dim3(256), 0, stream, rgb, h, w, tx, ty,
                       (int)(W != w), (int)(H != h), out, H, W, float3{mean[0], mean[1], mean[2]},
                       float3{stdv[0], stdv[1], stdv[2]});
    ODAM_HIP(hipGetLastError());
    return 0;
}

}
```

### odam_amd/csrc/detr_model.h

```cpp
#pragma once
#include <hip/hip_runtime.h>

#include <algorithm>
#include <map>
#include <string>
#include <utility>
#include <vector>

#include "../../include/odam_detr.h"
#include "cg_mx8.h"
#include "conv_gemm.h"
#include "odam_err.h"

namespace odam_dm {

struct HostTensor {
    std::vector<long long> shape;
    std::vector<float> data;
};

struct Conv {
    void* w = nullptr;
    void* w3 = nullptr;
    float* scale = nullptr;
// ... 53 lines not shown
        }
        return 0;
    }
};

}

struct odam_detr {
    odam_detr_cfg cfg;
    std::map<std::string, odam_dm::HostTensor> host;
    bool finalized = false;
    std::vector<void*> allocs;

    odam_dm::Conv stem;
    bool basic = false;
    int l4_ch = 2048;
    std::vector<odam_dm::Bottleneck> blocks;
    std::vector<int> block_stride;
    odam_dm::Conv input_proj;
    std::vector<odam_dm::EncLayer> enc;
    std::vector<odam_dm::DecLayer> dec;
    odam_dm::Conv cross_k_all, cross_v_all;
    odam_dm::LN dec_norm;
    odam_dm::LN enc_norm;
    const void* memory_out = nullptr;
    odam_dm::Conv class_embed;
    odam_dm::Conv mlp[5][3];
    odam_dm::Conv stem_rows;
    float* pos = nullptr;
    float* query_pos = nullptr;

    int H1, W1, H2, W2, fh, fw, L;

    char *x4 = nullptr, *stem_out = nullptr, *bufA = nullptr, *bufB = nullptr, *t1 = nullptr, *t2 = nullptr,
         *dsb = nullptr;
    char *src = nullptr, *srcpos = nullptr, *qk = nullptr, *v = nullptr, *att = nullptr, *tmp = nullptr, *ffn = nullptr;
    char *kc = nullptr, *vc = nullptr;
    char *tgt = nullptr, *tgtpos = nullptr, *dqk = nullptr, *dv = nullptr, *datt = nullptr, *dq = nullptr,
         *dtmp = nullptr, *dffn = nullptr, *hs = nullptr, *h1 = nullptr, *h2 = nullptr;
    const char* layer4 = nullptr;
    int es = 4;
    int dt = 0;
    bool mx = false;
    unsigned char *qa = nullptr, *qas = nullptr, *qb = nullptr, *qbs = nullptr, *qt1 = nullptr, *qt1s = nullptr, *qt2 = nullptr,
                  *qt2s = nullptr;

    odam_dm::EventLog conv_ev;
    odam_dm::EventLog att_ev;
    size_t stage_ev[6] = {};

    struct Resample { int* xmin; int* cnt; int* K; int ksize; };
    std::map<std::pair<int, int>, Resample> resample;

    template <typename T>
    int dev_alloc(T** p, size_t n) {
        ODAM_HIP(hipMalloc((void**)p, n * sizeof(T)));
        allocs.push_back((void*)*p);
        return 0;
    }
};

namespace odam_dm {

#define RC(call)                 \
    do {                         \
        int rc_ = (call);        \
        if (rc_) return rc_;     \
    } while (0)

odam_cg::ConvGemmArgs conv_args(const Conv& c, const void* x, int B, int H, int W, int dtype);
odam_mx::ConvArgs mx_args(const Conv& c, const void* x, const void* xs, int B, int H, int W);

int run_conv(const Conv& c, const void* x, int B, int H, int W, const void* res, bool relu, void* y, hipStream_t st,
             int dtype = 0, int out_f32 = 0);

}
```

### odam_amd/csrc/detr_ops.hip

```cpp
#include <hip/hip_runtime.h>

#include "detr_kernels.h"
#include "detr_model.h"

using namespace odam_dm;
using odam_cg::ConvGemmArgs;

namespace {

int fail(int code, const char* who, const char* what) {
    std::snprintf(g_odam_err, sizeof(g_odam_err), "%s: %s", who, what);
    return code;
}

int split_filters_for_call(const float* w_packed, int Cout, int Kpad, hipStream_t st, unsigned short** d3, const char* who) {
    *d3 = nullptr;
    if (!odam_cg::presplit_applies(Cout, Kpad)) return 0;
    std::vector<float> hw((size_t)Cout * Kpad);
    ODAM_HIP(hipStreamSynchronize(st));
    ODAM_HIP(hipMemcpy(hw.data(), w_packed, hw.size() * sizeof(float), hipMemcpyDeviceToHost));
    std::vector<unsigned short> h3(hw.size() * 3);
    odam_cg::split3_filters(hw.data(), Cout, Kpad, h3.data());
    ODAM_HIP(hipMalloc(d3, h3.size() * 2));
    if (hipMemcpy(*d3, h3.data(), h3.size() * 2, hipMemcpyHostToDevice) != hipSuccess) {
// ... 124 lines not shown
extern "C" int odam_op_conv2d_nhwc_mxfp8(const void* x, const void* xs, const void* w_packed, const void* ws, const float* scale,
                                         const float* bias, const void* residual, void* y, void* ys, void* y_bf16, float* y_f32,
                                         int B, int H, int W, int Cin, int Cout, int KH, int KW, int stride, int pad, int dil,
                                         int Kpad, int relu, int k_order, void* stream) {
    if (dil != 1) return odam_fail(1, "odam_op_conv2d_nhwc_mxfp8: dilation must be 1");
    if (k_order != 0) return odam_fail(1, "odam_op_conv2d_nhwc_mxfp8: k_order must be 0 (tap-major)");
    if (B < 1 || H < 1 || W < 1 || KH < 1 || KW < 1 || stride < 1 || pad < 0) return odam_fail(1, "odam_op_conv2d_nhwc_mxfp8: bad shape");
    Conv c = conv_of(nullptr, scale, bias, Cin, Cout, KH, KW, stride, pad, 1, Kpad, 0);
    c.wq = (unsigned char*)const_cast<void*>(w_packed); c.wqs = (unsigned char*)const_cast<void*>(ws);
    odam_mx::ConvArgs a = mx_args(c, x, xs, B, H, W);
    a.res = (const unsigned short*)residual; a.relu = relu ? 1 : 0;
    a.y = (unsigned char*)y; a.ys = (unsigned char*)ys; a.yb = (unsigned short*)y_bf16; a.yf = y_f32;
    return odam_mx::launch_conv(a, (hipStream_t)stream);
}

extern "C" int odam_op_bottleneck_bf16(const void* x, const void* w2, const float* s2, const float* b2, const void* w3,
                                       const float* s3, const float* b3, const void* residual, void* y, const void* w1n,
                                       const float* s1n, const float* b1n, void* y_next, int B, int H, int W, int P, int stride,
                                       int PN, void* stream) {
    if (!x || !w2 || !w3 || !y) return odam_fail(1, "odam_op_bottleneck_bf16: null pointer");
    ConvGemmArgs a = bottleneck_args(1, x, w2, s2, b2, s3, b3, residual, y, s1n, b1n, y_next, B, H, W, P, stride, w1n ? PN : 0);
    a.F_Wt = w3;
    if (w1n && PN > 0) a.G_Wt = w1n;
    if (!odam_cg::fused_bf16_ok(a)) return odam_fail(4, "odam_op_bottleneck_bf16: the fused kernel does not apply to this shape");
    return odam_cg::launch_conv_gemm(a, (hipStream_t)stream);
}

extern "C" int odam_op_bottleneck_f32(const float* x, const float* w2, const float* s2, const float* b2, const float* w3,
                                      const float* s3, const float* b3, const float* residual, float* y, const float* w1n,
                                      const float* s1n, const float* b1n, float* y_next, int B, int H, int W, int P, int stride,
                                      int PN, void* stream) {
    if (!x || !w2 || !w3 || !y) return odam_fail(1, "odam_op_bottleneck_f32: null pointer");
    if (PN > 0 && (!w1n || !y_next)) return odam_fail(1, "odam_op_bottleneck_f32: PN > 0 needs w1n and y_next");
    if (P != 64 && P != 128) return odam_fail(4, "odam_op_bottleneck_f32: the fused kernel is built for P = 64 and 128");
    hipStream_t st = (hipStream_t)stream;
    ConvGemmArgs a = bottleneck_args(0, x, w2, s2, b2, s3, b3, residual, y, s1n, b1n, y_next, B, H, W, P, stride, PN);
    a.Wt3 = w2; a.F_Wt3 = w3; a.G_Wt3 = PN > 0 ? w1n : nullptr;
    if (!odam_cg::fused_second_ok(a)) return odam_fail(4, "odam_op_bottleneck_f32: the fused kernel does not apply to this shape");
    unsigned short *d2 = nullptr, *d3 = nullptr, *d1 = nullptr;
    int rc = split_filters_for_call(w2, P, 9 * P, st, &d2, "odam_op_bottleneck_f32");
    if (!rc) rc = split_filters_for_call(w3, 4 * P, P, st, &d3, "odam_op_bottleneck_f32");
    if (!rc && PN > 0) rc = split_filters_for_call(w1n, PN, 4 * P, st, &d1, "odam_op_bottleneck_f32");
    if (!rc) {
        a.Wt3 = d2; a.F_Wt3 = d3; a.G_Wt3 = PN > 0 ? d1 : nullptr;
        rc = odam_cg::launch_conv_gemm(a, st);
    }
    (void)hipStreamSynchronize(st);
    if (d2) (void)hipFree(d2);
    if (d3) (void)hipFree(d3);
    if (d1) (void)hipFree(d1);
    return rc;
}

extern "C" long long odam_op_conv_paths(char* buf, int n, int reset) { return odam_cg::read_paths(buf, n, reset); }

extern "C" int odam_op_conv_bf16_mode(int mode) {
    if (mode < 0 || mode > 2) return odam_fail(1, "odam_op_conv_bf16_mode: mode must be 0, 1 or 2");
    odam_cg::set_big_mode(mode);
    return 0;
}

extern "C" int odam_op_conv_f32_mode(int mode) {
    if (mode != 0 && mode != 2) return odam_fail(1, "odam_op_conv_f32_mode: mode must be 0 or 2");
    odam_cg::set_f32_mode(mode);
    return 0;
}

extern "C" int odam_op_attention(const float* Q, int ldq, const float* K, int ldk, const float* V, int ldv, float* O,
                                 int ldo, int B, int H, int Lq, int Lk, void* stream) {
    return attention_op("odam_op_attention", ATT_NULLS, Q, ldq, K, ldk, V, ldv, O, ldo, B, H, Lq, Lk, 32, 0, nullptr, stream);
}

extern "C" int odam_op_attention_bf16(const void* Q, int ldq, const void* K, int ldk, const void* V, int ldv, void* O,
                                      int ldo, int B, int H, int Lq, int Lk, void* stream) {
    return attention_op("odam_op_attention_bf16", ATT_BF16, Q, ldq, K, ldk, V, ldv, O, ldo, B, H, Lq, Lk, 32, 1, nullptr, stream);
}

extern "C" int odam_op_attention_ex(const void* Q, int ldq, const void* K, int ldk, const void* V, int ldv, void* O, int ldo,
                                    int B, int H, int Lq, int Lk, int head_dim, int dtype, const unsigned char* key_mask,
                                    void* stream) {
    return attention_op("odam_op_attention_ex", ATT_EX, Q, ldq, K, ldk, V, ldv, O, ldo, B, H, Lq, Lk, head_dim, dtype, key_mask, stream);
}

extern "C" int odam_op_attention_hd(const void* Q, int ldq, const void* K, int ldk, const void* V, int ldv, void* O, int ldo,
                                    int B, int H, int Lq, int Lk, int head_dim, int dtype, const unsigned char* key_mask,
                                    void* stream) {
    return attention_op("odam_op_attention_hd", ATT_HD, Q, ldq, K, ldk, V, ldv, O, ldo, B, H, Lq, Lk, head_dim, dtype, key_mask, stream);
}

extern "C" int odam_op_add_layernorm(const float* x, const float* r, const float* gamma, const float* beta, float* y,
                                     int M, void* stream) {
    return layernorm_op("odam_op_add_layernorm", false, x, r, gamma, beta, y, nullptr, 1, nullptr, M, 256, 0, stream);
}

extern "C" int odam_op_add_layernorm_ex(const void* x, const void* r, const float* gamma, const float* beta, void* y,
                                        const float* pos, int L, void* y_pos, int M, int dtype, void* stream) {
    return layernorm_op("odam_op_add_layernorm_ex", true, x, r, gamma, beta, y, pos, L, y_pos, M, 256, dtype, stream);
}

extern "C" int odam_op_add_layernorm_c(const void* x, const void* r, const float* gamma, const float* beta, void* y,
                                       const float* pos, int L, void* y_pos, int M, int C, int dtype, void* stream) {
    return layernorm_op("odam_op_add_layernorm_c", true, x, r, gamma, beta, y, pos, L, y_pos, M, C, dtype, stream);
}

extern "C" int odam_op_maxpool3x3s2_nhwc_ex(const void* x, void* y, int B, int H, int W, int C, int dtype, void* stream) {
    return maxpool_op("odam_op_maxpool3x3s2_nhwc_ex", x, y, B, H, W, C, dtype, stream);
// ... 63 lines not shown
```

### odam_amd/csrc/detr_weights.hip

```cpp
#include <hip/hip_runtime.h>

#include <cmath>
#include <cstring>

#include "detr_model.h"

using namespace odam_dm;

namespace {

const HostTensor* find(odam_detr* m, const std::string& name) {
    auto it = m->host.find(name);
    return it == m->host.end() ? nullptr : &it->second;
}

#define NEED(var, name)                                                                    \
    const HostTensor* var = find(m, name);                                                 \
    if (!var) {                                                                            \
        std::snprintf(g_odam_err, sizeof(g_odam_err), "odam_detr_finalize: missing weight %s", std::string(name).c_str()); \
        return 1;                                                                          \
    }

int upload(odam_detr* m, float** p, const std::vector<float>& v) {
    if (int rc = m->dev_alloc(p, v.size())) return rc;
    ODAM_HIP(hipMemcpy(*p, v.data(), v.size() * sizeof(float), hipMemcpyHostToDevice));
    return 0;
}
int upload_u16(odam_detr* m, void** p, const std::vector<unsigned short>& h) {
    unsigned short* d = nullptr;
    if (int rc = m->dev_alloc(&d, h.size())) return rc;
    ODAM_HIP(hipMemcpy(d, h.data(), h.size() * 2, hipMemcpyHostToDevice));
    *p = d;
    return 0;
}
int upload_w3(odam_detr* m, void** p, const std::vector<float>& v, int Cout, int Kpad) {
    *p = nullptr;
    if (m->dt != 0 || Kpad % 16 != 0 || (long)Cout * Kpad * 6 >= 0x7fffffffL) return 0;
    std::vector<unsigned short> h((size_t)Cout * Kpad * 3);
    odam_cg::split3_filters(v.data(), Cout, Kpad, h.data());
    return upload_u16(m, p, h);
}
int upload_w(odam_detr* m, void** p, const std::vector<float>& v) {
    if (m->dt == 0) return upload(m, (float**)p, v);
    std::vector<unsigned short> h(v.size());
    for (size_t i = 0; i < v.size(); i++) {
        unsigned u;
        std::memcpy(&u, &v[i], 4);
        if ((u & 0x7fffffffu) > 0x7f800000u) h[i] = (unsigned short)((u >> 16) | 0x40);
        else h[i] = (unsigned short)((u + 0x7fffu + ((u >> 16) & 1u)) >> 16);
    }
    return upload_u16(m, p, h);
}

int pack_conv(odam_detr* m, Conv& c, const HostTensor& w, int stride, int pad, int dil = 1) {
    const int Cout = (int)w.shape[0], Cin = (int)w.shape[1];
    const int KH = w.shape.size() > 2 ? (int)w.shape[2] : 1, KW = w.shape.size() > 3 ? (int)w.shape[3] : 1;
    const int epc = m->dt ? 8 : 4;
    const int CinP = (Cin + epc - 1) / epc * epc;
// ... 41 lines not shown
    return m->mx ? pack_conv_mx(m, c, w, stride, pad) : pack_conv(m, c, w, stride, pad, dil);
}

int pack_linear(odam_detr* m, Conv& c, const HostTensor& w, const HostTensor* b, int r0, int r1) {
    const int K = (int)w.shape[1];
    std::vector<float> p(w.data.begin() + (size_t)r0 * K, w.data.begin() + (size_t)r1 * K);
    c.Cin = K; c.Cout = r1 - r0; c.KH = c.KW = 1; c.stride = 1; c.pad = 0; c.Kpad = K;
    if (int rc = upload_w3(m, &c.w3, p, r1 - r0, K)) return rc;
    if (int rc = upload_w(m, &c.w, p)) return rc;
    if (b) {
        std::vector<float> bb(b->data.begin() + r0, b->data.begin() + r1);
        if (int rc = upload(m, &c.bias, bb)) return rc;
    }
    return 0;
}

int fold_bn(odam_detr* m, Conv& c, const std::string& prefix) {
    NEED(w, prefix + ".weight"); NEED(b, prefix + ".bias");
    NEED(rm, prefix + ".running_mean"); NEED(rv, prefix + ".running_var");
    const size_t n = w->data.size();
    std::vector<float> sc(n), bi(n);
    for (size_t i = 0; i < n; i++) {
        const float s = w->data[i] * (1.0f / std::sqrt(rv->data[i] + 1e-5f));
        sc[i] = s;
        bi[i] = b->data[i] - rm->data[i] * s;
    }
    if (int rc = upload(m, &c.scale, sc)) return rc;
    return upload(m, &c.bias, bi);
}

int pack_ln(odam_detr* m, LN& ln, const std::string& prefix) {
    NEED(w, prefix + ".weight"); NEED(b, prefix + ".bias");
    if (w->data.size() != (size_t)m->cfg.hidden_dim || b->data.size() != (size_t)m->cfg.hidden_dim) {
        std::snprintf(g_odam_err, sizeof(g_odam_err), "odam_detr_finalize: %s must have hidden_dim = %d entries", prefix.c_str(),
                      m->cfg.hidden_dim);
        return 1;
    }
    if (int rc = upload(m, &ln.g, w->data)) return rc;
    return upload(m, &ln.b, b->data);
}

int check_in_proj(const HostTensor& w, const HostTensor& b, int E, const std::string& name) {
    if (w.shape.size() == 2 && w.shape[0] == 3LL * E && w.shape[1] == E && b.data.size() == 3 * (size_t)E) return 0;
    std::snprintf(g_odam_err, sizeof(g_odam_err), "odam_detr_finalize: %s.in_proj_weight must be [%d, %d] (hidden_dim %d)", name.c_str(),
                  3 * E, E, E);
    return 1;
}

int check_shape(const HostTensor& w, int cout, int cin, int k, const std::string& name) {
    if (w.shape.size() == 4 && w.shape[0] == cout && w.shape[1] == cin && w.shape[2] == k && w.shape[3] == k) return 0;
    std::snprintf(g_odam_err, sizeof(g_odam_err), "odam_detr_finalize: %s must be [%d, %d, %d, %d] for this backbone", name.c_str(),
                  cout, cin, k, k);
    return 1;
}

}

extern "C" int odam_detr_create(const odam_detr_cfg* cfg, odam_detr** out) {
    if (!cfg || !out) return odam_fail(1, "odam_detr_create: null argument");
    if (cfg->hidden_dim % 64 || cfg->hidden_dim < 128 || cfg->hidden_dim > 1024)
        return odam_fail(3, "odam_detr_create: hidden_dim must be a multiple of 64 in 128 .. 1024");
    if (cfg->nheads < 1 || cfg->hidden_dim % cfg->nheads)
        return odam_fail(3, "odam_detr_create: hidden_dim must be a multiple of nheads");
    if (cfg->hidden_dim / cfg->nheads != 32 && cfg->hidden_dim / cfg->nheads != 64)
        return odam_fail(3, "odam_detr_create: head dim hidden_dim / nheads must be 32 or 64 (16 and 128 are not built)");
    if (cfg->max_batch < 1 || cfg->img_h < 32 || cfg->img_w < 32) return odam_fail(1, "odam_detr_create: bad sizes");
    if (cfg->dtype < 0 || cfg->dtype > 2) return odam_fail(1, "odam_detr_create: dtype must be 0 (fp32), 1 (bf16) or 2 (mxfp8)");
    if (cfg->dtype == 2 && cfg->dilation)
        return odam_fail(3, "odam_detr_create: dilation (DC5) is not supported in the mxfp8 mode (dtype 2)");
    if (cfg->basic_block != 0 && cfg->basic_block != 1) return odam_fail(1, "odam_detr_create: basic_block must be 0 (Bottleneck) or 1 (BasicBlock)");
    if (cfg->basic_block && cfg->dilation)
        return odam_fail(3, "odam_detr_create: dilation (DC5) is not supported with BasicBlock backbones (resnet18 / resnet34)");
    for (int l = 0; l < 4; l++)
        if (cfg->resnet_blocks[l] < 1) return odam_fail(1, "odam_detr_create: every ResNet stage needs at least one block");
    odam_detr* m = new odam_detr();
    m->cfg = *cfg;
    m->basic = cfg->basic_block != 0;
    m->mx = cfg->dtype == 2;
    m->dt = cfg->dtype ? 1 : 0;
    m->es = cfg->dtype ? 2 : 4;
    m->H1 = conv_out(cfg->img_h, 7, 2, 3); m->W1 = conv_out(cfg->img_w, 7, 2, 3);
    m->H2 = conv_out(m->H1, 3, 2, 1); m->W2 = conv_out(m->W1, 3, 2, 1);
    int h = m->H2, w = m->W2;
    for (int l = 1; l < (cfg->dilation ? 3 : 4); l++) { h = conv_out(h, 3, 2, 1); w = conv_out(w, 3, 2, 1); }
    m->fh = h; m->fw = w; m->L = h * w;
    *out = m;
    return 0;
}

extern "C" int odam_detr_destroy(odam_detr* m) {
    if (!m) return 0;
    for (void* p : m->allocs) (void)hipFree(p);
    for (hipEvent_t e : m->conv_ev.ev) (void)hipEventDestroy(e);
    for (hipEvent_t e : m->att_ev.ev) (void)hipEventDestroy(e);
    delete m;
    return 0;
}

extern "C" int odam_detr_feature_hw(const odam_detr* m, int* h, int* w) {
    if (!m || !h || !w) return odam_fail(1, "odam_detr_feature_hw: null argument");
    *h = m->fh; *w = m->fw;
    return 0;
}

extern "C" int odam_detr_set_weight(odam_detr* m, const char* name, const float* data, const long long* shape,
                                    int ndim) {
    if (!m || !name || !data || (!shape && ndim > 0) || ndim < 0 || ndim > 4)
        return odam_fail(1, "odam_detr_set_weight: bad argument");
    if (m->finalized) return odam_fail(1, "odam_detr_set_weight: model already finalized");
    HostTensor t;
    size_t n = 1;
    for (int i = 0; i < ndim; i++) { t.shape.push_back(shape[i]); n *= (size_t)shape[i]; }
    t.data.assign(data, data + n);
    m->host[name] = std::move(t);
    return 0;
}

extern "C" int odam_detr_finalize(odam_detr* m) {
    if (!m) return odam_fail(1, "odam_detr_finalize: null model");
    if (m->finalized) return 0;
    const odam_detr_cfg& c = m->cfg;
    const std::string bb = "backbone.0.body.";
    {
        NEED(w, bb + "conv1.weight");
        RC(pack_conv(m, m->stem, *w, 2, 3));
        RC(fold_bn(m, m->stem, bb + "bn1"));
        {
            const int Cout = (int)w->shape[0];
            const int Kp = m->dt ? 256 : 224;
            std::vector<float> pr((size_t)Cout * Kp, 0.0f);
            for (int o = 0; o < Cout; o++)
                for (int ci = 0; ci < 3; ci++)
                    for (int ky = 0; ky < 7; ky++)
                        for (int kx = 0; kx < 7; kx++)
                            pr[(size_t)o * Kp + ky * 32 + kx * 4 + ci] = w->data[(((size_t)o * 3 + ci) * 7 + ky) * 7 + kx];
            Conv& r = m->stem_rows;
            r.Cin = 32; r.Cout = Cout; r.KH = 7; r.KW = 1; r.stride = 2; r.pad = 0; r.Kpad = Kp; r.k_order = m->dt ? 0 : 1;
            RC(upload_w3(m, &r.w3, pr, Cout, Kp));
            RC(upload_w(m, &r.w, pr));
            r.scale = m->stem.scale; r.bias = m->stem.bias;
        }
    }
    int inplanes = 64;
    for (int l = 0; l < 4; l++) {
        for (int i = 0; i < c.resnet_blocks[l]; i++) {
            const std::string p = bb + "layer" + std::to_string(l + 1) + "." + std::to_string(i) + ".";
            if (m->basic) {
                const int planes = 64 << l, stride = (i == 0 && l > 0) ? 2 : 1;
                const bool ds = stride != 1 || inplanes != planes;
                Bottleneck b;
                NEED(w1, p + "conv1.weight"); NEED(w2, p + "conv2.weight");
                RC(check_shape(*w1, planes, inplanes, 3, p + "conv1.weight"));
                RC(check_shape(*w2, planes, planes, 3, p + "conv2.weight"));
                RC(pack_body(m, b.c1, *w1, stride, 1)); RC(fold_bn(m, b.c1, p + "bn1"));
                RC(pack_body(m, b.c2, *w2, 1, 1)); RC(fold_bn(m, b.c2, p + "bn2"));
                if (ds) {
                    NEED(wd, p + "downsample.0.weight");
                    RC(check_shape(*wd, planes, inplanes, 1, p + "downsample.0.weight"));
                    RC(pack_body(m, b.ds, *wd, stride, 0)); RC(fold_bn(m, b.ds, p + "downsample.1"));
                    b.has_ds = true;
                }
                m->blocks.push_back(b);
                m->block_stride.push_back(stride);
                inplanes = planes;
                continue;
            }
            const bool dc5 = c.dilation && l == 3;
            const int stride = (i == 0 && l > 0 && !dc5) ? 2 : 1;
            const int dil = (dc5 && i > 0) ? 2 : 1;
            Bottleneck b;
            NEED(w1, p + "conv1.weight"); NEED(w2, p + "conv2.weight"); NEED(w3, p + "conv3.weight");
            RC(pack_body(m, b.c1, *w1, 1, 0));
            RC(pack_body(m, b.c2, *w2, stride, dil, dil));
            RC(pack_body(m, b.c3, *w3, 1, 0));
            RC(fold_bn(m, b.c1, p + "bn1")); RC(fold_bn(m, b.c2, p + "bn2")); RC(fold_bn(m, b.c3, p + "bn3"));
            if (i == 0) {
                NEED(wd, p + "downsample.0.weight");
                RC(pack_body(m, b.ds, *wd, stride, 0)); RC(fold_bn(m, b.ds, p + "downsample.1"));
                b.has_ds = true;
            }
            m->blocks.push_back(b);
            m->block_stride.push_back(stride);
        }
    }
    m->l4_ch = m->basic ? m->blocks.back().c2.Cout : m->blocks.back().c3.Cout;
    {
        NEED(w, "input_proj.weight"); NEED(b, "input_proj.bias");
        if (w->shape.size() != 4 || (int)w->shape[1] != m->l4_ch) {
            std::snprintf(g_odam_err, sizeof(g_odam_err), "odam_detr_finalize: input_proj.weight must read the layer4 map (%d channels for "
                          "this backbone)", m->l4_ch);
            return 1;
        }
        RC(pack_conv(m, m->input_proj, *w, 1, 0));
        RC(upload(m, &m->input_proj.bias, b->data));
// ... 102 lines not shown
```

### odam_amd/csrc/odam_common.hip

```cpp
#include <atomic>
#include <cstdio>
#include <cstring>

#include "odam_config.h"
#include "odam_err.h"

extern "C" const char* odam_last_error(void) { return g_odam_err; }

namespace odam_cfg {
namespace {
struct Entry { const char* name; int def, lo, hi; };
const Entry TABLE[N_KEYS] = {
    {"cg.ring", 1, 0, 2},        {"cg.f32", 2, 0, 2},         {"cg.fuse", 2, 0, 2},       {"cg.fuse_bf16", 2, 0, 2},
    {"cg.s1", 1, 0, 1},          {"cg.ut", 1, 0, 1},          {"cg.tiles", 31, 0, 31},      {"cg.force", 0, 0, 3},
    {"cg.presplit", 1, 0, 1},    {"cg.mfma16", 3, 0, 3},      {"att.x3", 1, 0, 1},         {"att.bf16_mfma", 1, 0, 1}, {"stem.rows", 1, 0, 1},
    {"assoc.persist", 2, 0, 2},  {"sq.split", 32, 1, 32},     {"sq.split_wait", 3000, 0, 100000000}, {"sq.lanes", 0, 0, 64},
    {"stem.pool", 1, 0, 1},
    {"cg.pin", 0, 0, 1},
    {"cg.small_x3", 1, 0, 1},
    {"assoc.sk_fast", 1, 0, 3},
    {"assoc.hungarian", 0, 0, 1},
    {"assoc.merge", 1, 0, 1},
    {"sq.two_per_cu", 1, 0, 1},
};
std::atomic<int> g_val[N_KEYS];
std::atomic<bool> g_init{false};
void init() {
    if (g_init.load(std::memory_order_acquire)) return;
    for (int k = 0; k < N_KEYS; k++) g_val[k].store(TABLE[k].def, std::memory_order_relaxed);
    g_init.store(true, std::memory_order_release);
}
}
int get(Key k) { init(); return g_val[k].load(std::memory_order_relaxed); }
void set(Key k, int v) { init(); g_val[k].store(v, std::memory_order_relaxed); }
}

extern "C" int odam_config_set(const char* key, int value) {
    using namespace odam_cfg;
    if (!key) return odam_fail(1, "odam_config_set: null key");
    for (int k = 0; k < N_KEYS; k++)
        if (std::strcmp(key, TABLE[k].name) == 0) {
            if (value < TABLE[k].lo || value > TABLE[k].hi || (k == CG_F32 && value == 1)) {
                std::snprintf(g_odam_err, sizeof(g_odam_err), "odam_config_set: %s = %d outside %d..%d", key, value, TABLE[k].lo, TABLE[k].hi);
                return 1;
            }
            set((Key)k, value);
            return 0;
        }
    std::snprintf(g_odam_err, sizeof(g_odam_err), "odam_config_set: unknown key %s", key);
    return 1;
}

extern "C" int odam_config_get(const char* key, int* value) {
    using namespace odam_cfg;
    if (!key || !value) return odam_fail(1, "odam_config_get: null pointer");
    for (int k = 0; k < N_KEYS; k++)
        if (std::strcmp(key, TABLE[k].name) == 0) { *value = get((Key)k); return 0; }
    std::snprintf(g_odam_err, sizeof(g_odam_err), "odam_config_get: unknown key %s", key);
    return 1;
}

extern "C" int odam_config_describe(char* buf, int n) {
    using namespace odam_cfg;
    if (!buf || n <= 0) return odam_fail(1, "odam_config_describe: bad buffer");
    int pos = 0;
    buf[0] = 0;
    for (int k = 0; k < N_KEYS; k++) {
        const int v = get((Key)k);
        const int w = std::snprintf(buf + pos, (size_t)(n - pos), "%s%s=%d%s", k ? " " : "", TABLE[k].name, v, v != TABLE[k].def ? "*" : "");
        if (w < 0 || w >= n - pos) return odam_fail(1, "odam_config_describe: buffer too small");
        pos += w;
    }
    return 0;
}
```

### odam_amd/csrc/odam_config.h

```cpp
#pragma once

namespace odam_cfg {
enum Key {
    CG_RING,
    CG_F32,
    CG_FUSE,
    CG_FUSE_BF16,
    CG_S1,
    CG_UT,
    CG_TILES,
    CG_FORCE,
    CG_PRESPLIT,
    CG_MFMA16,
    ATT_X3,
    ATT_BF16_MFMA,
    STEM_ROWS,
    ASSOC_PERSIST,
    SQ_SPLIT,
    SQ_SPLIT_WAIT,
    SQ_LANES,
    STEM_POOL,
    CG_PIN,
    CG_SMALL_X3,
    ASSOC_SK_FAST,
    ASSOC_HUNGARIAN,
    ASSOC_MERGE,
    SQ_TWO_PER_CU,
    N_KEYS
};
int get(Key k);
void set(Key k, int v);
}
```

### odam_amd/detector.py

```python
import ctypes
import math
import numbers

import numpy as np
import torch

from . import _lib
from .weights import RESNET_BLOCK_TYPE, RESNET_BLOCKS, layer4_channels


class _Cfg(ctypes.Structure):
    _fields_ = [("resnet_blocks", ctypes.c_int * 4), ("hidden_dim", ctypes.c_int), ("nheads", ctypes.c_int),
                ("dim_feedforward", ctypes.c_int), ("enc_layers", ctypes.c_int), ("dec_layers", ctypes.c_int),
                ("num_queries", ctypes.c_int), ("num_classes1", ctypes.c_int), ("angle_bins", ctypes.c_int),
                ("max_batch", ctypes.c_int), ("img_h", ctypes.c_int), ("img_w", ctypes.c_int), ("dtype", ctypes.c_int),
                ("pre_norm", ctypes.c_int), ("dilation", ctypes.c_int), ("basic_block", ctypes.c_int)]


def _axis_phase_table(counts, channels, temperature):
    pair = torch.arange(channels, dtype=torch.float32).div(2, rounding_mode="floor")
    wavelength = torch.pow(float(temperature), pair * 2 / channels)
    phase = counts.unsqueeze(-1) / wavelength
    table = torch.empty_like(phase)
    table[..., 0::2] = torch.sin(phase[..., 0::2])
# ... 51 lines not shown


def _forward_aux_entry():
    f = _lib.lib().odam_detr_forward_aux
    if f.argtypes is None:
        f.argtypes, f.restype = FORWARD_AUX_ARGTYPES, ctypes.c_int
    return f


def _select_pack_entry():
    f = _lib.lib().odam_detr_select_pack
    if f.argtypes is None:
        f.argtypes, f.restype = SELECT_PACK_ARGTYPES, ctypes.c_int
    return f


class Detector:

    def __init__(self, backbone="resnet50", hidden_dim=256, nheads=8, dim_feedforward=2048, enc_layers=6,
                 dec_layers=6, num_queries=100, num_classes=18, angle_bins=30, max_batch=8, device="cuda:0",
                 n_streams=2, dtype="fp32", pre_norm=False, position_embedding="sine", dilation=False):
        self.n_streams = max(1, int(n_streams))
        if backbone not in RESNET_BLOCKS:
            raise ValueError(f"backbone={backbone!r}: not supported (one of {', '.join(sorted(RESNET_BLOCKS))})")
        self.basic_block = RESNET_BLOCK_TYPE[backbone] == "basic"
        if self.basic_block and dilation:
            raise ValueError(f"backbone={backbone!r}: dilation (DC5) is not supported with BasicBlock backbones")
        if position_embedding not in ("sine", "v2", "learned", "v3"):
            raise ValueError(f"not supported {position_embedding}")
        self.learned_pos = position_embedding in ("learned", "v3")
        self.pre_norm = bool(pre_norm)
        self.dilation = bool(dilation)
        self.resize = (800, 1333)
        if dtype not in ("fp32", "bf16", "mxfp8"):
            raise ValueError("dtype must be 'fp32' (parity mode), 'bf16' (BASELINE config 4) or 'mxfp8' (MXFP8 ResNet body)")
        if dtype == "mxfp8" and dilation:
            raise ValueError("dtype='mxfp8': dilation (DC5) is not supported in the mxfp8 mode")
        check_transformer_width(hidden_dim, nheads)
        self.dtype = dtype
        self.arch = dict(backbone=backbone, hidden_dim=hidden_dim, nheads=nheads, dim_feedforward=dim_feedforward,
                         enc_layers=enc_layers, dec_layers=dec_layers, num_queries=num_queries,
                         num_classes1=num_classes + 1, angle_bins=angle_bins)
        self.num_queries = num_queries
        self.max_batch = max_batch
        self.device = torch.device(device)
        self._sd = None
        self._handles = {}
        self._sincos_dev = {}

    def to(self, device):
        new = torch.device("cuda:0" if str(device) == "cuda" else device)
        if new != self.device:
            self.close()
            for name in ("_streams", "_mscratch", "_xform", "_stage", "_copy_stream", "_pinned"):
                if hasattr(self, name):
                    setattr(self, name, None)
        self.device = new
        return self

    def cuda(self):
        return self.to("cuda:0")

    def eval(self):
        return self

    def load_state_dict(self, state_dict, strict=True):
        self._sd = {k: v.detach().to("cpu", torch.float32).contiguous() for k, v in state_dict.items()
                    if torch.is_tensor(v) and not k.endswith("num_batches_tracked")}
        self.close()
        return self

    def close(self):
        for h in self._handles.values():
            _lib.lib().odam_detr_destroy(h)
        self._handles = {}
        self._streams = None

    def __del__(self):
        try:
            self.close()
        except Exception:
            pass

    def _handle(self, H, W, idx=0):
        key = (H, W, idx)
        if key in self._handles:
            return self._handles[key]
        if self._sd is None:
            raise _lib.OdamError("Detector: load_state_dict() must be called before the first forward")
        L = _lib.lib()
        a = self.arch
        cfg = _Cfg()
        for i, n in enumerate(RESNET_BLOCKS[a["backbone"]]):
            cfg.resnet_blocks[i] = n
        for k in ("hidden_dim", "nheads", "dim_feedforward", "enc_layers", "dec_layers", "num_queries", "num_classes1",
                  "angle_bins"):
            setattr(cfg, k, a[k])
        cfg.max_batch, cfg.img_h, cfg.img_w = self.max_batch, H, W
        cfg.dtype = {"fp32": 0, "bf16": 1, "mxfp8": 2}[self.dtype]
        cfg.pre_norm = 1 if self.pre_norm else 0
        cfg.dilation = 1 if self.dilation else 0
        cfg.basic_block = 1 if self.basic_block else 0
        h = ctypes.c_void_p()
        with torch.cuda.device(self.device):
            _lib.check(L.odam_detr_create(ctypes.byref(cfg), ctypes.byref(h)), "odam_detr_create")
            try:
                self._fill_handle(h)
# ... 88 lines not shown

    def __call__(self, samples, aux=False):
        if isinstance(samples, (list, tuple)):
            if len({tuple(t.shape) for t in samples}) > 1:
                return self.forward_nested(samples, aux=aux)
            samples = torch.stack(list(samples))
        x = samples.to(self.device, torch.float32).contiguous()
        B, C, H, W = x.shape
        assert C == 3
        h = self._handle(H, W)
        if aux:
            blocks = self._layer_blocks(B)
            for b0 in range(0, B, self.max_batch):
                b1 = min(B, b0 + self.max_batch)
                self._forward_layers(h, x[b0:b1], blocks, b0, b1)
            return self._layer_dict(blocks, H, W)
        a = self.arch
        Q = a["num_queries"]
        dev = self.device
        mk = lambda n: torch.empty(B, Q, n, device=dev, dtype=torch.float32)
        out = {"pred_logits": mk(a["num_classes1"]), "pred_boxes": mk(4), "pred_angle": mk(a["angle_bins"]),
               "pred_offset": mk(2), "pred_size": mk(3), "pred_depth": mk(1), "pred_obj_features": mk(a["hidden_dim"])}
        L = _lib.lib()
        stream = torch.cuda.current_stream(dev).cuda_stream
        with torch.cuda.device(dev):
            for b0 in range(0, B, self.max_batch):
                b1 = min(B, b0 + self.max_batch)
                sl = lambda t: _lib.ptr(t[b0:b1])
                _lib.check(L.odam_detr_forward(h, _lib.ptr(x[b0:b1]), ctypes.c_int(b1 - b0), sl(out["pred_logits"]),
                                               sl(out["pred_boxes"]), sl(out["pred_angle"]), sl(out["pred_offset"]),
                                               sl(out["pred_size"]), sl(out["pred_depth"]),
                                               sl(out["pred_obj_features"]), ctypes.c_void_p(stream)),
                           "odam_detr_forward")
        out["_hw"] = (H, W)
        return out

    forward = __call__

    def preprocess_u8(self, rgb, out=None, idx=0, stream=None):
        from .transforms import MEAN, STD, target_size
        B, h, w, c = rgb.shape
        assert c == 3 and rgb.dtype == torch.uint8 and rgb.is_cuda and rgb.is_contiguous()
        H, W = target_size(w, h, *self.resize)
        if out is None:
            out = torch.empty(B, 3, H, W, device=self.device, dtype=torch.float32)
        st = stream if stream is not None else torch.cuda.current_stream(self.device).cuda_stream
        mean, std = (ctypes.c_float * 3)(*MEAN), (ctypes.c_float * 3)(*STD)
        with torch.cuda.device(self.device):
            _lib.check(_lib.lib().odam_detr_preprocess_u8(self._handle(H, W, idx), _lib.ptr(rgb), ctypes.c_int(B),
                                                          ctypes.c_int(h), ctypes.c_int(w), mean, std, _lib.ptr(out),
                                                          ctypes.c_void_p(st)), "odam_detr_preprocess_u8")
        return out

    def forward_u8(self, rgb):
        outs = [self(self.preprocess_u8(rgb[b0:b0 + self.max_batch])) for b0 in range(0, rgb.shape[0], self.max_batch)]
        if len(outs) == 1:
            return outs[0]
        res = {k: torch.cat([o[k] for o in outs]) for k in outs[0] if k != "_hw"}
        res["_hw"] = outs[0]["_hw"]
        return res

    def debug_taps(self, B, H, W):
        hd = self._handle(H, W)
        L = _lib.lib()
        fh, fw = ctypes.c_int(), ctypes.c_int()
        L.odam_detr_feature_hw(hd, ctypes.byref(fh), ctypes.byref(fw))
        l4 = torch.empty(B, layer4_channels(self.arch["backbone"]), fh.value, fw.value, device=self.device)
        mem = torch.empty(B, fh.value * fw.value, self.arch["hidden_dim"], device=self.device)
        with torch.cuda.device(self.device):
            _lib.check(L.odam_detr_debug_read(hd, B, _lib.ptr(l4), _lib.ptr(mem),
                                              ctypes.c_void_p(torch.cuda.current_stream(self.device).cuda_stream)),
                       "odam_detr_debug_read")
        return l4, mem

    def postprocess_rows(self, out, img_size, intr_mat, on_device=False):
        H, W = out["_hw"]
        h = self._handle(H, W)
        B = out["pred_logits"].shape[0]
        rows = torch.empty(B, self.num_queries, 16, device=self.device, dtype=torch.float32)
        K9 = np.ascontiguousarray(np.asarray(intr_mat, np.float64)[:3, :3], np.float32)
        img_w, img_h = img_size
        with torch.cuda.device(self.device):
            _lib.check(_lib.lib().odam_detr_postprocess(
                h, _lib.ptr(out["pred_logits"]), _lib.ptr(out["pred_boxes"]), _lib.ptr(out["pred_angle"]),
                _lib.ptr(out["pred_offset"]), _lib.ptr(out["pred_size"]), _lib.ptr(out["pred_depth"]), ctypes.c_int(B),
                K9.ctypes.data_as(_lib.c_float_p), ctypes.c_float(img_w), ctypes.c_float(img_h), _lib.ptr(rows),
                ctypes.c_void_p(torch.cuda.current_stream(self.device).cuda_stream)), "odam_detr_postprocess")
        if on_device:
            return rows
        return rows.cpu().numpy()

    @staticmethod
    def select(rows, threshold, nms_2d=True, n_bins=30):
        rows = np.ascontiguousarray(rows, np.float32)
        Q = rows.shape[0]
        keep = np.zeros(max(Q, 1), np.int32)
        n = ctypes.c_int()
        _lib.check(_lib.lib().odam_detr_select(rows.ctypes.data_as(_lib.c_float_p), ctypes.c_int(Q),
                                               ctypes.c_float(threshold), ctypes.c_int(int(bool(nms_2d))),
                                               keep.ctypes.data_as(_lib.c_int_p), ctypes.byref(n)), "odam_detr_select")
        r = rows[keep[:n.value]]
        return dict(bboxes=r[:, 2:6].reshape(-1, 2, 2).copy(), dimensions=r[:, 10:13].copy(),
                    angles=(r[:, 9] * np.float32(180 / n_bins)).astype(np.float32), translates=r[:, 6:9].copy(),
                    classes=r[:, 1].astype(np.int64), scores=r[:, 0].copy())

    def _sincos(self):
        cache = self._sincos_dev
        key = (str(self.device), self.arch["angle_bins"])
        if key not in cache:
            cache[key] = torch.from_numpy(sincos_table(self.arch["angle_bins"])).to(self.device)
        return cache[key]

    def _frame_ids_dev(self, frame_ids):
# ... 25 lines not shown
        dev = self.device
        pack = dict(frame_ids=self._frame_ids_dev(frame_ids), seq_size=seq_size, threshold=threshold, nms_2d=nms_2d,
                    out=(torch.empty(N, 30, 15, device=dev, dtype=torch.float32), torch.empty(N, device=dev, dtype=torch.int32)))
        assert pack["frame_ids"].shape == (N,)
        self._sincos()
        for _ in self.detect_resident_chunks(frames, img_size, intr_mat, chunk=1 << 30, batch=batch, _pack=pack):
            pass
        return pack["out"]

    def detect_resident(self, frames, img_size, intr_mat):
        out = np.empty((frames.shape[0], self.num_queries, 16), np.float32)
        for c0, rows in self.detect_resident_chunks(frames, img_size, intr_mat, chunk=1 << 30):
            out[c0:c0 + rows.shape[0]] = rows
        return out

    @staticmethod
    def batch_for(n_frames):
        return 42 if n_frames <= 300 else 38

    def detect_resident_chunks(self, frames, img_size, intr_mat, chunk=128, batch=None, _pack=None):
        raw = frames.dtype == torch.uint8
        if raw:
            from .transforms import target_size
            N, H, W = frames.shape[0], *target_size(frames.shape[2], frames.shape[1], *self.resize)
        else:
            N, _, H, W = frames.shape
        a = self.arch
        Q = a["num_queries"]
        dev = self.device
        L = _lib.lib()
        mb = self.max_batch
        bb = mb if not batch else min(mb, self.batch_for(N) if batch == "auto" else int(batch))
        ns = self.n_streams
        handles = [self._handle(H, W, k) for k in range(ns)]
        chunk = max(bb, (chunk // bb) * bb)
        rows = torch.empty(N, Q, 16, device=dev, dtype=torch.float32)
        if _pack is None and (getattr(self, "_pinned", None) is None or self._pinned.shape[0] < N):
            self._pinned = torch.empty(N, Q, 16, dtype=torch.float32, pin_memory=True)
        host = self._pinned[:N] if _pack is None else None
        if getattr(self, "_streams", None) is None or len(self._streams) != ns:
            self._streams = [torch.cuda.Stream(device=dev) for _ in range(ns)]
            mk = lambda n: torch.empty(mb, Q, n, device=dev, dtype=torch.float32)
            self._mscratch = [[mk(a["num_classes1"]), mk(4), mk(a["angle_bins"]), mk(2), mk(3), mk(1)] for _ in range(ns)]
        K9 = np.ascontiguousarray(np.asarray(intr_mat, np.float64)[:3, :3], np.float32)
        img_w, img_h = img_size
        main = torch.cuda.current_stream(dev)
        start = torch.cuda.Event()
        start.record(main)
        for st in self._streams:
            st.wait_event(start)
        events = []
        nb = 0
        on_host = not frames.is_cuda
        if raw:
            if getattr(self, "_xform", None) is None or self._xform[0].shape[2:] != (H, W) or len(self._xform) != ns:
                self._xform = [torch.empty(mb, 3, H, W, device=dev, dtype=torch.float32) for _ in range(ns)]
        if on_host:
            st0 = getattr(self, "_stage", None)
            if st0 is None or st0[0][0].shape[1:] != frames.shape[1:] or st0[0][0].dtype != frames.dtype or len(st0) != ns:
                self._stage = [[torch.empty((mb,) + tuple(frames.shape[1:]), device=dev, dtype=frames.dtype)
                                for _ in range(2)] for _ in range(ns)]
                self._copy_stream = torch.cuda.Stream(device=dev)
            stage_free = [[None, None] for _ in range(ns)]
        with torch.cuda.device(dev):
            for c0 in range(0, N, chunk):
                c1 = min(N, c0 + chunk)
                used = set()
                for b0 in range(c0, c1, bb):
                    B = min(bb, c1 - b0)
                    k = nb % ns
                    nb += 1
                    used.add(k)
                    lg, bx, an, of, sz, dp = self._mscratch[k]
                    sp = ctypes.c_void_p(self._streams[k].cuda_stream)
                    src = frames[b0:b0 + B]
                    if on_host:
                        j = ((nb - 1) // ns) & 1
                        buf = self._stage[k][j][:B]
                        if stage_free[k][j] is not None:
                            self._copy_stream.wait_event(stage_free[k][j])
                        with torch.cuda.stream(self._copy_stream):
                            buf.copy_(src, non_blocking=True)
                            up = torch.cuda.Event()
                            up.record(self._copy_stream)
                        self._streams[k].wait_event(up)
                        src = buf
                    if raw:
                        src = self.preprocess_u8(src, self._xform[k][:B], k, self._streams[k].cuda_stream)
                    _lib.check(L.odam_detr_forward(handles[k], _lib.ptr(src), ctypes.c_int(B), _lib.ptr(lg),
                                                   _lib.ptr(bx), _lib.ptr(an), _lib.ptr(of), _lib.ptr(sz), _lib.ptr(dp),
                                                   ctypes.c_void_p(0), sp), "odam_detr_forward")
                    _lib.check(L.odam_detr_postprocess(handles[k], _lib.ptr(lg), _lib.ptr(bx), _lib.ptr(an), _lib.ptr(of),
                                                       _lib.ptr(sz), _lib.ptr(dp), ctypes.c_int(B),
                                                       K9.ctypes.data_as(_lib.c_float_p), ctypes.c_float(img_w),
                                                       ctypes.c_float(img_h), _lib.ptr(rows[b0:b0 + B]), sp),
                               "odam_detr_postprocess")
                    if _pack is not None:
                        self.select_pack(rows[b0:b0 + B], _pack["frame_ids"][b0:b0 + B], _pack["seq_size"], _pack["threshold"],
                                         _pack["nms_2d"], out=(_pack["out"][0][b0:b0 + B], _pack["out"][1][b0:b0 + B]),
                                         stream=self._streams[k].cuda_stream)
                    if on_host:
                        stage_free[k][j] = torch.cuda.Event()
                        stage_free[k][j].record(self._streams[k])
                for k in used:
                    e = torch.cuda.Event()
                    e.record(self._streams[k])
                    main.wait_event(e)
                if _pack is not None:
                    continue
                host[c0:c1].copy_(rows[c0:c1], non_blocking=True)
                ev = torch.cuda.Event()
                ev.record(main)
                events.append((c0, c1, ev))
        for c0, c1, ev in events:
            ev.synchronize()
            yield c0, host[c0:c1].numpy().copy()

    def profile(self, H, W, on):
        _lib.check(_lib.lib().odam_detr_profile_enable(self._handle(H, W), ctypes.c_int(int(on))), "profile_enable")

    def profile_read(self, H, W):
        n, ms, fl = ctypes.c_int(), ctypes.c_double(), ctypes.c_double()
        _lib.check(_lib.lib().odam_detr_profile_read(self._handle(H, W), ctypes.byref(n), ctypes.byref(ms),
                                                     ctypes.byref(fl)), "profile_read")
        return n.value, ms.value, fl.value

    def profile_read_attention(self, H, W):
        n, ms, fl = ctypes.c_int(), ctypes.c_double(), ctypes.c_double()
        _lib.check(_lib.lib().odam_detr_profile_read_attention(self._handle(H, W), ctypes.byref(n), ctypes.byref(ms),
                                                               ctypes.byref(fl)), "profile_read_attention")
        return n.value, ms.value, fl.value

    def profile_read_stages(self, H, W):
        n = (ctypes.c_int * 6)()
        ms, fl = (ctypes.c_double * 6)(), (ctypes.c_double * 6)()
        _lib.check(_lib.lib().odam_detr_profile_read_stages(self._handle(H, W), ctypes.c_int(6), n, ms, fl), "profile_read_stages")
        names = ("stem", "layer1", "layer2", "layer3", "layer4", "rest")
        return {k: (n[i], ms[i], fl[i]) for i, k in enumerate(names)}

    def postprocess(self, out, img_size, threshold, intr_mat, nms_2d=True):
        rows = self.postprocess_rows(out, img_size, intr_mat)
        res = {k: [] for k in ("bboxes", "dimensions", "angles", "translates", "classes", "scores")}
        for b in range(rows.shape[0]):
            s = self.select(rows[b], threshold, nms_2d, self.arch["angle_bins"])
# ... 22 lines not shown
```

Baseline: 1120.

## Fuse u8 preprocessing into stem conv via bf16 activation plane and folded normalization

```diff
diff --git a/include/odam_detr.h b/include/odam_detr.h
--- a/include/odam_detr.h
+++ b/include/odam_detr.h
@@ -59,6 +59,10 @@
 int odam_detr_preprocess_u8(odam_detr* m, const unsigned char* rgb, int B, int h, int w, const float* mean,
                             const float* std_dev, float* out, void* stream);
 
+int odam_detr_forward_u8(odam_detr* m, const unsigned char* rgb, int B, int h, int w, const float* mean, const float* std_dev,
+                         float* logits, float* boxes, float* angle, float* offset, float* size, float* depth, float* obj_features,
+                         void* stream);
+
 int odam_detr_profile_enable(odam_detr* m, int on);
 int odam_detr_profile_read(odam_detr* m, int* n_launches, double* total_ms, double* total_flops);
 int odam_detr_profile_read_attention(odam_detr* m, int* n_launches, double* total_ms, double* total_flops);
@@ -85,6 +89,8 @@
 int odam_op_conv_bf16_mode(int mode);
 int odam_op_conv_f32_mode(int mode);
 long long odam_op_pooled_stem_launches(void);
+int odam_op_stem_u8(const unsigned char* rgb, int B, int h, int w, int H, int W, const float* conv1_w, const float* scale,
+                    const float* bias, const float* mean, const float* std_dev, float* y, int* path, void* stream);
 int odam_op_attention(const float* Q, int ldq, const float* K, int ldk, const float* V, int ldv, float* O, int ldo,
                       int B, int H, int Lq, int Lk, void* stream);
 int odam_op_attention_bf16(const void* Q, int ldq, const void* K, int ldk, const void* V, int ldv, void* O, int ldo,
diff --git a/odam_amd/_lib.py b/odam_amd/_lib.py
--- a/odam_amd/_lib.py
+++ b/odam_amd/_lib.py
@@ -61,6 +61,8 @@
     "odam_assoc_ot_batch": [_P, _P, _P, _P, _P, _I, _I, _F, _I, _P, _P, _P, _P, _P, _P, _P],
     "odam_assoc_reserve_batch": [_P, _I, _I],
     "odam_assoc_forward_batch": [_P, _P, _P, _P, _P, _I, _P, _P, _P, _P, _P, _P, _P],
+    "odam_detr_forward_u8": [_P, _P, _I, _I, _I, _P, _P, _P, _P, _P, _P, _P, _P, _P, _P],
+    "odam_op_stem_u8": [_P, _I, _I, _I, _I, _I, _P, _P, _P, _P, _P, _P, _P, _P],
 }
 
 
diff --git a/odam_amd/csrc/cg_args.h b/odam_amd/csrc/cg_args.h
--- a/odam_amd/csrc/cg_args.h
+++ b/odam_amd/csrc/cg_args.h
@@ -41,6 +41,7 @@
     int pool = 0, pool_ph = 0, pool_pw = 0, Hp = 0, Wp = 0;
     int no_pin = 0;
     int s1_window = 0;
+    int a_bf16 = 0;
 };
 
 constexpr int POOL_PH = 8, POOL_PW = 14;
diff --git a/odam_amd/csrc/cg_big.hpp b/odam_amd/csrc/cg_big.hpp
--- a/odam_amd/csrc/cg_big.hpp
+++ b/odam_amd/csrc/cg_big.hpp
@@ -22,7 +22,7 @@
     const int ring = NST * (MODE >= 3 ? bm * 64 + 96 * BN : (bm + BN) * 64);
     const int wm = big_wm(MODE, BN, NTH);
     const int wn = NTH / 64 / wm;
-    const int slab = MODE == 4 ? (NTH / 64) * 16 * ((BN / wn > 128 ? 128 : BN / wn) + 4) * 4 : (NTH / 64) * 32 * (BN / wn) * 4;
+    const int slab = MODE >= 4 ? (NTH / 64) * 16 * ((BN / wn > 128 ? 128 : BN / wn) + 4) * 4 : (NTH / 64) * 32 * (BN / wn) * 4;
     const int s1 = (MODE == 0 && NTH == 512) ? (BN == 256 ? 2 : (BN == 128 ? 3 : 4)) * (384 * 64 + 3 * BN * 64) : 0;
     const int m = ring > slab ? ring : slab;
     const int deep = big_deep_a(MODE, BN, NST, NTH) ? (6 + 4) * 256 * 64 : 0;
@@ -36,12 +36,17 @@
                       (FUSE >= 5 && FUSE <= 8 && MODE == 0 && NTH == 512 && NST == 4),
                   "fused layers: pre-split filters with 64-column tiles (FUSE 1, 2, 4) or 128-column tiles (FUSE 3); bf16 (FUSE 5 + "
                   "log2(PN / 32), 5 = no chained reduce)");
-    static_assert(MODE == 0 || MODE == 2 || MODE == 3 || MODE == 4,
-                  "bf16 operands, fp32 split, fp32 split with pre-split filters (3: 32x32x16 matrix instruction, 4: 16x16x32)");
+    static_assert(MODE == 0 || MODE == 2 || MODE == 3 || MODE == 4 || MODE == 5,
+                  "bf16 operands, fp32 split, fp32 split with pre-split filters (3: 32x32x16 matrix instruction, 4: 16x16x32, 5: 16x16x32 "
+                  "with the activations as ONE bf16 plane in memory)");
     static_assert(MODE != 4 || FUSE <= 4, "the 16x16x32 schedule: its own epilogue, or the fp32 bottleneck tails");
     constexpr bool BF16 = MODE == 0;
-    constexpr bool PRE = MODE == 3 || MODE == 4;
-    constexpr bool X16 = MODE == 4;
+    constexpr bool PRE = MODE == 3 || MODE == 4 || MODE == 5;
+    constexpr bool X16 = MODE == 4 || MODE == 5;
+    constexpr bool A16 = MODE == 5;
+    static_assert(!A16 || (NTH == 1024 && BN == 64 && FUSE == 0), "bf16 activations: the sixteen-wave 512 x 64 tile only");
+    constexpr int AES = A16 ? 2 : (int)sizeof(typename std::conditional<BF16, unsigned short, float>::type);
+    constexpr int AEPC = 16 / AES;
     static_assert(!PRE || NTH == 512 || (X16 && NTH == 1024), "pre-split filters: eight-wave workgroups, or sixteen waves (16x16x32 loop)");
     static_assert(NTH != 1024 || (FUSE == 0 && ((BN == 64 && (X16 || BF16)) || (BN == 256 && BF16))), "sixteen waves: plain layers (512 x 64: bf16 or the 16x16x32 split loop; 256 x 256: bf16)");
     using T = typename std::conditional<BF16, unsigned short, float>::type;
@@ -77,7 +82,7 @@
     }
     const int tile_m = bid / tiles_n, tile_n = bid - tile_m * tiles_n;
     const int m0 = tile_m * BM, n0 = tile_n * BN;
-    constexpr bool POOLABLE = NTH == 1024 && BN == 64 && FUSE == 0 && (MODE == 4 || MODE == 0);
+    constexpr bool POOLABLE = NTH == 1024 && BN == 64 && FUSE == 0 && (X16 || MODE == 0);
     constexpr int pl_tw = 2 * POOL_PW + 1, pl_rows = (2 * POOL_PH + 1) * pl_tw;
     static_assert(pl_rows <= 512, "a patch fits a 512-row tile");
     int pl_b = 0, pl_y0 = 0, pl_x0 = 0;
@@ -129,9 +134,10 @@
     const int kw_inv = (65536 + a.KW - 1) / a.KW;
     const int nt_inv = (65536 + ntaps - 1) / ntaps;
     const int b0 = (POOLABLE && a.pool) ? pl_b : m0 / hw;
-    const int csrc = X16 ? (c4 ^ ((lane >> 4) & 1)) : (c4 ^ ((lane >> 4) & 3));
+    const int csrc = A16 ? (c4 ^ ((0 - (lane >> 4)) & 3))
+                   : X16 ? (c4 ^ ((lane >> 4) & 1)) : (c4 ^ ((lane >> 4) & 3));
     const int margin = (a.pad * a.W + a.pad) * lda;
-    const unsigned long long pa = (unsigned long long)(Ag + (size_t)b0 * a.H * a.W * lda - margin), pw = (unsigned long long)Wg;
+    const unsigned long long pa = (unsigned long long)a.A + ((size_t)b0 * a.H * a.W * lda - (size_t)margin) * AES, pw = (unsigned long long)Wg;
     const u32x4 a_rs4 = u32x4{(unsigned)pa, (unsigned)(pa >> 32) & 0xffffu, OOB_VOFF, 0x00020000u};
     const u32x4 w_rs4 = u32x4{(unsigned)pw, (unsigned)(pw >> 32) & 0xffffu, OOB_VOFF, 0x00020000u};
     unsigned a_voff[A_LD], a_mask[A_LD], w_voff[B_LD];
@@ -153,7 +159,7 @@
             iy0 = oy * a.stride - a.pad; ix0 = ox * a.stride - a.pad;
             base = ((b * a.H + iy0) * a.W + ix0) * lda;
         }
-        a_voff[i] = (unsigned)(base - b0 * a.H * a.W * lda + margin + csrc * EPC) * (unsigned)sizeof(T);
+        a_voff[i] = (unsigned)(base - b0 * a.H * a.W * lda + margin + csrc * AEPC) * (unsigned)AES;
         unsigned mk = plain ? 1u : 0u;
         for (int t = 0; t < (plain ? 0 : ntaps); t++) {
             const int ky = (t * kw_inv) >> 16, kx = t - ky * a.KW;
@@ -346,8 +352,9 @@
             const TilePrep tp = tile_prep(kt);
 #pragma unroll
             for (int part = 0; part < A_LD; part++) {
+                if (A16 && (kt & 1)) break;
                 const unsigned vo = ((a_mask[part] >> tp.tap) & 1u) ? a_voff[part] : OOB_VOFF;
-                lds_dma16(a_rs4, lds_base + (unsigned)(st * STAGE + wave_u * 16 * ROWB + RPP * part * ROWB), vo, tp.soff_a);
+                lds_dma16(a_rs4, lds_base + (unsigned)(st * STAGE + wave_u * 16 * ROWB + RPP * part * ROWB), vo, A16 ? tp.soff_a >> 1 : tp.soff_a);
             }
 #pragma unroll
             for (int j = 0; j < B3_HI; j++)
@@ -361,7 +368,7 @@
             const TilePrep tp = tile_prep(kt);
             if (part < A_LD) {
                 const unsigned vo = ((a_mask[part] >> tp.tap) & 1u) ? a_voff[part] : OOB_VOFF;
-                lds_dma16(a_rs4, lds_base + (unsigned)(st * STAGE + wave_u * 16 * ROWB + RPP * part * ROWB), vo, tp.soff_a);
+                lds_dma16(a_rs4, lds_base + (unsigned)(st * STAGE + wave_u * 16 * ROWB + RPP * part * ROWB), vo, A16 ? tp.soff_a >> 1 : tp.soff_a);
             } else {
                 const int j = part - A_LD;
                 if (j + 1 < B3_HI || b_wave)
@@ -383,6 +390,41 @@
         unsigned long long st_acc[4] = {0, 0, 0, 0}, st_prev = __builtin_readcyclecounter();
         const unsigned long long st_loop0 = st_prev;
 #endif
+        if constexpr (A16) {
+            const int a5_lane = (wm * (BM / WM) + r16) * ROWB + ((kq ^ ((0 - (r16 >> 2)) & 3)) << 4);
+            constexpr int NA5 = A_LD, NDMA5 = NA5 + 2 * B3_HI, NBLK5 = MI * NJ;
+            for (int kp = 0; 2 * kp < nk; ++kp) {
+                asm volatile("s_waitcnt vmcnt(0)" ::: "memory");
+                __builtin_amdgcn_s_barrier();
+                asm volatile("" ::: "memory");
+                const int s0 = (2 * kp) & 3;
+                const char* Sa = lds_c + s0 * STAGE + a5_lane;
+                const char* Sb = lds_c + s0 * STAGE + b_lane;
+                uint4 av[MI], bh[NJ], bm[NJ], bl[NJ];
+#pragma unroll
+                for (int mi = 0; mi < MI; mi++) av[mi] = *reinterpret_cast<const uint4*>(Sa + mi * 16 * ROWB);
+#pragma unroll
+                for (int j = 0; j < NJ; j++) {
+                    const char* bp = Sb + j * 16 * 32;
+                    bh[j] = *reinterpret_cast<const uint4*>(bp);
+                    bm[j] = *reinterpret_cast<const uint4*>(bp + BN * 32);
+                    bl[j] = *reinterpret_cast<const uint4*>(bp + 2 * BN * 32);
+                }
+                int dpart = 0;
+#pragma unroll
+                for (int b = 0; b < NBLK5; b++) {
+                    const int mi = b / NJ, nj = b % NJ;
+                    ODAM_MM16(c16[mi][nj], av[mi], bh[nj]); ODAM_MM16(c16[mi][nj], av[mi], bm[nj]); ODAM_MM16(c16[mi][nj], av[mi], bl[nj]);
+#pragma unroll
+                    for (; dpart < ((b + 1) * NDMA5 + NBLK5 - 1) / NBLK5; dpart++) {
+                        const int half_ = dpart < NA5 ? 0 : (dpart - NA5) / B3_HI;
+                        const int part = dpart < NA5 ? dpart : A_LD + (dpart - NA5) % B3_HI;
+                        dma_part16(2 * kp + 2 + half_, (s0 ^ 2) + half_, part);
+                    }
+                    __builtin_amdgcn_sched_barrier(0);
+                }
+            }
+        } else
         for (int kp = 0; 2 * kp < nk; ++kp) {
             CG_STAMP_AT(3);
             asm volatile("s_waitcnt vmcnt(0)" ::: "memory");
@@ -1021,7 +1063,7 @@
     constexpr int bm = big_bm(BN, NTH);
     int tiles = ((a.M + bm - 1) / bm) * ((a.Cout + BN - 1) / BN);
     if (a.pool) {
-        if (!(NTH == 1024 && BN == 64 && (MODE == 4 || MODE == 0)) || a.Cout != 64 || a.pool_ph != POOL_PH || a.pool_pw != POOL_PW ||
+        if (!(NTH == 1024 && BN == 64 && (MODE == 4 || MODE == 5 || MODE == 0)) || a.Cout != 64 || a.pool_ph != POOL_PH || a.pool_pw != POOL_PW ||
             a.ldc != a.Cout || a.res)
             return odam_fail(1, "conv_gemm: pooled stem asked for where it does not apply");
         tiles = a.B * ((a.Hp + POOL_PH - 1) / POOL_PH) * ((a.Wp + POOL_PW - 1) / POOL_PW);
diff --git a/odam_amd/csrc/cg_big_f32.hip b/odam_amd/csrc/cg_big_f32.hip
--- a/odam_amd/csrc/cg_big_f32.hip
+++ b/odam_amd/csrc/cg_big_f32.hip
@@ -5,6 +5,7 @@
 int launch_big_f32(int mode, int bn, int nth, const ConvGemmArgs& a, hipStream_t stream) {
     if (nth == 1024) {
         if (mode == 4 && bn == 64) return launch_big<4, 64, 4, 1024>(a, 0, stream);
+        if (mode == 5 && bn == 64) return launch_big<5, 64, 4, 1024>(a, 0, stream);
     } else if (bn == 256) {
         if (mode == 4) return launch_big<4, 256, 4>(a, 0, stream);
         if (mode == 3) return launch_big<3, 256, 4>(a, 0, stream);
diff --git a/odam_amd/csrc/cg_choice.h b/odam_amd/csrc/cg_choice.h
--- a/odam_amd/csrc/cg_choice.h
+++ b/odam_amd/csrc/cg_choice.h
@@ -32,6 +32,8 @@
 bool fused_second_ok(const ConvGemmArgs& a, const Switches& sw);
 bool fused_bf16_ok(const ConvGemmArgs& a, const Switches& sw);
 bool pooled_stem_ok(const ConvGemmArgs& a, const Switches& sw);
+bool bf16_plane_ok(const ConvGemmArgs& a, const Switches& sw);
+bool bf16_plane_ok(const ConvGemmArgs& a);
 bool fused_second_ok(const ConvGemmArgs& a);
 bool fused_bf16_ok(const ConvGemmArgs& a);
 bool pooled_stem_ok(const ConvGemmArgs& a);
diff --git a/odam_amd/csrc/cg_choice.hip b/odam_amd/csrc/cg_choice.hip
--- a/odam_amd/csrc/cg_choice.hip
+++ b/odam_amd/csrc/cg_choice.hip
@@ -125,7 +125,17 @@
     return ring_eligible(a, sw, 64) && fills_512_row_tiles(a, sw);
 }
 
+bool bf16_plane_ok(const ConvGemmArgs& a, const Switches& sw) {
+    if (is_bf16(a) || !sw.ring || !(sw.tiles & 8) || ring_mode_f32(a, sw) != 4) return false;
+    if (a.Cout <= 32 || a.Cout > 64 || a.Cin % 32 != 0 || a.res) return false;
+    const long lda = a.lda > 0 ? a.lda : a.Cin;
+    if ((lda * a.stride * 2) % 16 != 0 || (lda * a.W * 2) % 16 != 0 || (lda * a.pad * 2) % 16 != 0) return false;
+    if (a.pool && !pooled_stem_ok(a, sw)) return false;
+    return ring_eligible(a, sw, 64) && fills_512_row_tiles(a, sw);
+}
+
 bool fused_second_ok(const ConvGemmArgs& a) { return fused_second_ok(a, current_switches()); }
+bool bf16_plane_ok(const ConvGemmArgs& a) { return bf16_plane_ok(a, current_switches()); }
 bool fused_bf16_ok(const ConvGemmArgs& a) { return fused_bf16_ok(a, current_switches()); }
 bool pooled_stem_ok(const ConvGemmArgs& a) { return pooled_stem_ok(a, current_switches()); }
 bool presplit_applies(int Cout, int Kpad) { return f32_mode() == 2 && split_planes_fit(Cout, Kpad); }
@@ -139,6 +149,10 @@
         return refuse("conv_gemm: k_order 1 needs Cin % k-tile == 0, at most 32 taps, fewer than 2048 k-tiles");
     if (a.M <= 0 || a.Cout <= 0) return Choice{};
 
+    if (a.a_bf16) {
+        if (!bf16_plane_ok(a, sw)) return refuse("conv_gemm: bf16-plane activations asked for where they do not apply (check bf16_plane_ok)");
+        return ring(a, sw, 5, 64, 16);
+    }
     if (a.pool) {
         if (!pooled_stem_ok(a, sw)) return refuse("conv_gemm: pooled stem asked for where it does not apply (check pooled_stem_ok)");
         return ring(a, sw, bf ? 0 : 4, 64, 16);
diff --git a/odam_amd/csrc/detr_forward.hip b/odam_amd/csrc/detr_forward.hip
--- a/odam_amd/csrc/detr_forward.hip
+++ b/odam_amd/csrc/detr_forward.hip
@@ -103,6 +103,15 @@
                             [&] { return odam_cg::launch_conv_gemm(a, st); });
 }
 
+ConvGemmArgs stem_u8_args(odam_detr* m, int B, const void* w3, bool pool) {
+    ConvGemmArgs a = conv_args(m->stem_rows, m->x4, B, m->cfg.img_h + 6, m->cfg.img_w + 8, 0);
+    a.Wt3 = w3; a.a_bf16 = 1;
+    a.lda = 4; a.Ho = m->H1; a.Wo = m->W1; a.M = B * a.Ho * a.Wo;
+    a.relu = 1; a.C = m->stem_out;
+    if (pool) { a.pool = 1; a.pool_ph = odam_cg::POOL_PH; a.pool_pw = odam_cg::POOL_PW; a.Hp = m->H2; a.Wp = m->W2; a.C = m->bufA; }
+    return a;
+}
+
 int mx_t(odam_detr* m, const Conv& c, const unsigned char* x, const unsigned char* xs, int B, int H, int W, const void* res, bool relu,
          unsigned char* y, unsigned char* ys, void* yb, hipStream_t st) {
     odam_mx::ConvArgs a = mx_args(c, x, xs, B, H, W);
@@ -130,12 +139,8 @@
 
 int stem(odam_detr* m, const float* img, int B, hipStream_t st) {
     const int dt = m->dt, ih = m->cfg.img_h, iw = m->cfg.img_w;
-    const bool rows_ok = odam_cfg::get(odam_cfg::STEM_ROWS) != 0;
     bool pooled = false;
-    const long Mst = (long)B * m->H1 * m->W1;
-    const bool rows_mode = dt ? (m->stem_rows.w != nullptr && odam_cfg::get(odam_cfg::CG_RING) != 0)
-                              : (m->stem_rows.w3 != nullptr && odam_cg::f32_mode() == 2);
-    if (rows_ok && rows_mode && (Mst >= 192L * 256 || odam_cfg::get(odam_cfg::CG_PIN))) {
+    if (stem_rows_applies(m, B)) {
         RC(odam_dk::launch_nchw_to_nhwc4_framed(img, m->x4, B, ih, iw, dt, st));
         RC(stem_rows_t(m, B, st, m->bufA, &pooled));
     } else {
@@ -145,6 +150,47 @@
     if (!pooled) RC(odam_dk::launch_maxpool3x3s2(m->stem_out, m->bufA, B, m->H1, m->W1, 64, m->H2, m->W2, dt, st));
     return 0;
 }
+
+}
+
+namespace odam_dm {
+
+bool stem_rows_applies(const odam_detr* m, int B) {
+    const long Mst = (long)B * m->H1 * m->W1;
+    const bool rows_mode = m->dt ? (m->stem_rows.w != nullptr && odam_cfg::get(odam_cfg::CG_RING) != 0)
+                                 : (m->stem_rows.w3 != nullptr && odam_cg::f32_mode() == 2);
+    return odam_cfg::get(odam_cfg::STEM_ROWS) != 0 && rows_mode && (Mst >= 192L * 256 || odam_cfg::get(odam_cfg::CG_PIN));
+}
+
+int stem_from_u8(odam_detr* m, const unsigned char* rgb, int B, int h, int w, const float* mean, const float* stdv, hipStream_t st, int* path) {
+    const int ih = m->cfg.img_h, iw = m->cfg.img_w;
+    odam_detr::Resample tx{}, ty{};
+    RC(resample_tables(m, h, w, &tx, &ty));
+    if (path) *path = 0;
+    if (odam_cfg::get(odam_cfg::STEM_U8) != 0 && m->dt == 0 && !m->mx && (iw + 8) % 2 == 0 && !m->conv1_w.empty() && stem_rows_applies(m, B)) {
+        bool pooled = odam_cg::bf16_plane_ok(stem_u8_args(m, B, m->stem_rows.w3, true));
+        if (pooled || odam_cg::bf16_plane_ok(stem_u8_args(m, B, m->stem_rows.w3, false))) {
+            const odam_detr::StemU8* f = nullptr;
+            RC(stem_u8_filters(m, mean, stdv, &f));
+            RC(odam_dk::launch_preprocess_u8_bf16x4_framed(rgb, B, h, w, tx.xmin, tx.cnt, tx.K, tx.ksize, ty.xmin, ty.cnt, ty.K, ty.ksize,
+                                                           m->x4, ih, iw, f->centre, st));
+            const ConvGemmArgs a = stem_u8_args(m, B, f->w3, pooled);
+            if (pooled) g_pooled_stem_launches.fetch_add(1);
+            RC(m->conv_ev.timed(st, 2.0 * a.M * (double)a.Cout * 147, [&] { return odam_cg::launch_conv_gemm(a, st); }));
+            if (!pooled) RC(odam_dk::launch_maxpool3x3s2(m->stem_out, m->bufA, B, m->H1, m->W1, 64, m->H2, m->W2, 0, st));
+            if (path) *path = 1;
+            return 0;
+        }
+    }
+    if (!m->u8_img) RC(m->dev_alloc(&m->u8_img, (size_t)m->cfg.max_batch * 3 * ih * iw));
+    RC(odam_dk::launch_preprocess_u8(rgb, B, h, w, tx.xmin, tx.cnt, tx.K, tx.ksize, ty.xmin, ty.cnt, ty.K, ty.ksize, m->u8_img, ih, iw, mean,
+                                     stdv, st));
+    return stem(m, m->u8_img, B, st);
+}
+
+}
+
+namespace {
 
 int body_mxfp8(odam_detr* m, int B, Act& s, hipStream_t st) {
     unsigned char *cq = m->qa, *cs = m->qas, *nq = m->qb, *ns = m->qbs;
@@ -322,17 +368,20 @@
     return 0;
 }
 
+struct RawFrames { const unsigned char* rgb; int h, w; const float *mean, *stdv; };
+
 int forward_impl(odam_detr* m, const float* img, int B, const unsigned char* key_mask, const float* pos_b,
                  float* logits, float* boxes, float* angle, float* offset, float* size, float* depth,
-                 float* obj_features, void* stream, int frames_per_layer = 0) {
-    if (!m || !img || !logits || !boxes || !angle || !offset || !size || !depth)
+                 float* obj_features, void* stream, int frames_per_layer = 0, const RawFrames* raw = nullptr) {
+    if (!m || (!img && !raw) || !logits || !boxes || !angle || !offset || !size || !depth)
         return odam_fail(1, "odam_detr_forward: null pointer");
     if (!m->finalized) return odam_fail(1, "odam_detr_forward: call odam_detr_finalize first");
     if (B < 1 || B > m->cfg.max_batch) return odam_fail(3, "odam_detr_forward: batch outside 1..max_batch");
     hipStream_t st = (hipStream_t)stream;
     m->conv_ev.used = m->att_ev.used = 0;
 
-    RC(stem(m, img, B, st));
+    if (raw) RC(stem_from_u8(m, raw->rgb, B, raw->h, raw->w, raw->mean, raw->stdv, st, nullptr));
+    else RC(stem(m, img, B, st));
     std::fill(m->stage_ev, m->stage_ev + 6, m->conv_ev.used);
     m->stage_ev[0] = 0;
     Act s{m->bufA, m->bufB, m->H2, m->W2};
@@ -362,6 +411,15 @@
 extern "C" int odam_detr_forward(odam_detr* m, const float* img, int B, float* logits, float* boxes, float* angle,
                                  float* offset, float* size, float* depth, float* obj_features, void* stream) {
     return forward_impl(m, img, B, nullptr, nullptr, logits, boxes, angle, offset, size, depth, obj_features, stream);
+}
+
+extern "C" int odam_detr_forward_u8(odam_detr* m, const unsigned char* rgb, int B, int h, int w, const float* mean, const float* stdv,
+                                    float* logits, float* boxes, float* angle, float* offset, float* size, float* depth,
+                                    float* obj_features, void* stream) {
+    if (!rgb || !mean || !stdv) return odam_fail(1, "odam_detr_forward_u8: null pointer");
+    if (h < 1 || w < 1) return odam_fail(1, "odam_detr_forward_u8: bad size");
+    const RawFrames raw{rgb, h, w, mean, stdv};
+    return forward_impl(m, nullptr, B, nullptr, nullptr, logits, boxes, angle, offset, size, depth, obj_features, stream, 0, &raw);
 }
 
 extern "C" int odam_detr_forward_masked(odam_detr* m, const float* img, int B, const unsigned char* key_mask,
diff --git a/odam_amd/csrc/detr_input.hip b/odam_amd/csrc/detr_input.hip
--- a/odam_amd/csrc/detr_input.hip
+++ b/odam_amd/csrc/detr_input.hip
@@ -49,6 +49,11 @@
     m->resample[{in_size, out_size}] = t;
     *r = t;
     return 0;
+}
+
+int odam_dm::resample_tables(odam_detr* m, int h, int w, odam_detr::Resample* tx, odam_detr::Resample* ty) {
+    RC(resample_table(m, w, m->cfg.img_w, tx));
+    return resample_table(m, h, m->cfg.img_h, ty);
 }
 
 extern "C" int odam_detr_preprocess_u8(odam_detr* m, const unsigned char* rgb, int B, int h, int w, const float* mean,
diff --git a/odam_amd/csrc/detr_kernels.h b/odam_amd/csrc/detr_kernels.h
--- a/odam_amd/csrc/detr_kernels.h
+++ b/odam_amd/csrc/detr_kernels.h
@@ -31,6 +31,9 @@
                        const float* size, const float* depth, int B, int Q, int n_cls1, int n_bins, float img_w,
                        float img_h, float fx, float fy, float cx, float cy, float* rows, hipStream_t stream);
 
+int launch_preprocess_u8_bf16x4_framed(const unsigned char* rgb, int B, int h, int w, const int* tx_xmin, const int* tx_cnt,
+                                       const int* tx_K, int tx_ksize, const int* ty_xmin, const int* ty_cnt, const int* ty_K,
+                                       int ty_ksize, void* out, int H, int W, const int centre[3], hipStream_t stream);
 int launch_preprocess_u8(const unsigned char* rgb, int B, int h, int w, const int* tx_xmin, const int* tx_cnt,
                          const int* tx_K, int tx_ksize, const int* ty_xmin, const int* ty_cnt, const int* ty_K,
                          int ty_ksize, float* out, int H, int W, const float mean[3], const float stdv[3],
diff --git a/odam_amd/csrc/detr_kernels.hip b/odam_amd/csrc/detr_kernels.hip
--- a/odam_amd/csrc/detr_kernels.hip
+++ b/odam_amd/csrc/detr_kernels.hip
@@ -4,6 +4,7 @@
 
 #include "odam_config.h"
 #include "odam_err.h"
+#include "stem_u8_fold.h"
 
 namespace odam_dk {
 
@@ -937,15 +938,8 @@
     return v < 0 ? 0 : (v > 255 ? 255 : v);
 }
 
-__global__ __launch_bounds__(256) void preprocess_u8_kernel(const unsigned char* __restrict__ rgb, int h, int w,
-                                                            ResampleTable tx, ResampleTable ty, int need_x, int need_y,
-                                                            float* __restrict__ out, int H, int W, float3 mean,
-                                                            float3 stdv) {
-    const int X = blockIdx.x * 256 + threadIdx.x;
-    const int Y = blockIdx.y;
-    const size_t b = blockIdx.z;
-    if (X >= W) return;
-    const unsigned char* img = rgb + b * (size_t)h * w * 3;
+__device__ __forceinline__ void resample_u8_pixel(const unsigned char* __restrict__ img, int w, const ResampleTable& tx, const ResampleTable& ty,
+                                                  int need_x, int need_y, int X, int Y, int& u0, int& u1, int& u2) {
     const int x0 = need_x ? tx.xmin[X] : X, nx = need_x ? tx.cnt[X] : 1;
     const int y0 = need_y ? ty.xmin[Y] : Y, ny = need_y ? ty.cnt[Y] : 1;
     const int* kx = tx.K + (size_t)X * tx.ksize;
@@ -971,9 +965,21 @@
         }
         last[0] = hv[0]; last[1] = hv[1]; last[2] = hv[2];
     }
-    const int u0 = need_y ? clip8_22(acc[0]) : last[0];
-    const int u1 = need_y ? clip8_22(acc[1]) : last[1];
-    const int u2 = need_y ? clip8_22(acc[2]) : last[2];
+    u0 = need_y ? clip8_22(acc[0]) : last[0];
+    u1 = need_y ? clip8_22(acc[1]) : last[1];
+    u2 = need_y ? clip8_22(acc[2]) : last[2];
+}
+
+__global__ __launch_bounds__(256) void preprocess_u8_kernel(const unsigned char* __restrict__ rgb, int h, int w,
+                                                            ResampleTable tx, ResampleTable ty, int need_x, int need_y,
+                                                            float* __restrict__ out, int H, int W, float3 mean,
+                                                            float3 stdv) {
+    const int X = blockIdx.x * 256 + threadIdx.x;
+    const int Y = blockIdx.y;
+    const size_t b = blockIdx.z;
+    if (X >= W) return;
+    int u0, u1, u2;
+    resample_u8_pixel(rgb + b * (size_t)h * w * 3, w, tx, ty, need_x, need_y, X, Y, u0, u1, u2);
     const size_t plane = (size_t)H * W, o = (b * 3 * H + Y) * (size_t)W + X;
     out[o] = ((float)u0 / 255.0f - mean.x) / stdv.x;
     out[o + plane] = ((float)u1 / 255.0f - mean.y) / stdv.y;
@@ -993,4 +999,32 @@
     return 0;
 }
 
-}
+__global__ __launch_bounds__(256) void preprocess_u8_bf16x4_framed_kernel(const unsigned char* __restrict__ rgb, int h, int w,
+                                                                          ResampleTable tx, ResampleTable ty, int need_x, int need_y,
+                                                                          uint2* __restrict__ out, int H, int W, int c0, int c1, int c2) {
+    const int Xp = blockIdx.x * 256 + threadIdx.x;
+    const int Yp = blockIdx.y;
+    const size_t b = blockIdx.z;
+    if (Xp >= W + 8) return;
+    int X, Y;
+    uint2 v = uint2{0u, 0u};
+    if (odam_dm::stem_u8_inside(Xp, Yp, H, W, X, Y)) {
+        int u0, u1, u2;
+        resample_u8_pixel(rgb + b * (size_t)h * w * 3, w, tx, ty, need_x, need_y, X, Y, u0, u1, u2);
+        odam_dm::stem_u8_pixel(u0, u1, u2, c0, c1, c2, v.x, v.y);
+    }
+    out[(b * (H + 6) + Yp) * (size_t)(W + 8) + Xp] = v;
+}
+
+int launch_preprocess_u8_bf16x4_framed(const unsigned char* rgb, int B, int h, int w, const int* tx_xmin, const int* tx_cnt,
+                                       const int* tx_K, int tx_ksize, const int* ty_xmin, const int* ty_cnt, const int* ty_K,
+                                       int ty_ksize, void* out, int H, int W, const int centre[3], hipStream_t stream) {
+    if (B <= 0) return 0;
+    ResampleTable tx{tx_xmin, tx_cnt, tx_K, tx_ksize}, ty{ty_xmin, ty_cnt, ty_K, ty_ksize};
+    hipLaunchKernelGGL(preprocess_u8_bf16x4_framed_kernel, dim3((W + 8 + 255) / 256, H + 6, B), dim3(256), 0, stream, rgb, h, w, tx, ty,
+                       (int)(W != w), (int)(H != h), (uint2*)out, H, W, centre[0], centre[1], centre[2]);
+    ODAM_HIP(hipGetLastError());
+    return 0;
+}
+
+}
diff --git a/odam_amd/csrc/detr_model.h b/odam_amd/csrc/detr_model.h
--- a/odam_amd/csrc/detr_model.h
+++ b/odam_amd/csrc/detr_model.h
@@ -129,6 +129,11 @@
     struct Resample { int* xmin; int* cnt; int* K; int ksize; };
     std::map<std::pair<int, int>, Resample> resample;
 
+    struct StemU8 { float mean[3], stdv[3]; int centre[3]; void* w3; };
+    std::vector<float> conv1_w;
+    std::vector<StemU8> stem_u8;
+    float* u8_img = nullptr;
+
     template <typename T>
     int dev_alloc(T** p, size_t n) {
         ODAM_HIP(hipMalloc((void**)p, n * sizeof(T)));
@@ -148,6 +153,12 @@
 odam_cg::ConvGemmArgs conv_args(const Conv& c, const void* x, int B, int H, int W, int dtype);
 odam_mx::ConvArgs mx_args(const Conv& c, const void* x, const void* xs, int B, int H, int W);
 
+int pack_stem_rows(odam_detr* m, const float* w, int Cout, float* scale, float* bias);
+int stem_u8_filters(odam_detr* m, const float* mean, const float* stdv, const odam_detr::StemU8** out);
+int resample_tables(odam_detr* m, int h, int w, odam_detr::Resample* tx, odam_detr::Resample* ty);
+int stem_from_u8(odam_detr* m, const unsigned char* rgb, int B, int h, int w, const float* mean, const float* stdv, hipStream_t st, int* path);
+bool stem_rows_applies(const odam_detr* m, int B);
+
 int run_conv(const Conv& c, const void* x, int B, int H, int W, const void* res, bool relu, void* y, hipStream_t st,
              int dtype = 0, int out_f32 = 0);
 
diff --git a/odam_amd/csrc/detr_ops.hip b/odam_amd/csrc/detr_ops.hip
--- a/odam_amd/csrc/detr_ops.hip
+++ b/odam_amd/csrc/detr_ops.hip
@@ -200,6 +200,33 @@
     return rc;
 }
 
+extern "C" int odam_op_stem_u8(const unsigned char* rgb, int B, int h, int w, int H, int W, const float* conv1_w, const float* scale,
+                               const float* bias, const float* mean, const float* std_dev, float* y, int* path, void* stream) {
+    const char* who = "odam_op_stem_u8";
+    if (!rgb || !conv1_w || !scale || !bias || !mean || !std_dev || !y) return fail(1, who, "null pointer");
+    if (B < 1 || h < 1 || w < 1 || H < 32 || W < 32) return fail(1, who, "bad size");
+    hipStream_t st = (hipStream_t)stream;
+    odam_detr m{};
+    m.cfg.img_h = H; m.cfg.img_w = W; m.cfg.max_batch = B;
+    m.H1 = conv_out(H, 7, 2, 3); m.W1 = conv_out(W, 7, 2, 3);
+    m.H2 = conv_out(m.H1, 3, 2, 1); m.W2 = conv_out(m.W1, 3, 2, 1);
+    auto run = [&]() -> int {
+        RC(pack_stem_rows(&m, conv1_w, 64, const_cast<float*>(scale), const_cast<float*>(bias)));
+        if (!stem_rows_applies(&m, B)) return fail(4, who, "conv1 does not run as the row convolution here");
+        RC(m.dev_alloc(&m.x4, (size_t)B * (H + 6) * (W + 8) * 16));
+        RC(m.dev_alloc(&m.stem_out, (size_t)B * m.H1 * m.W1 * 64 * 4));
+        m.bufA = reinterpret_cast<char*>(y);
+        int p = 0;
+        RC(stem_from_u8(&m, rgb, B, h, w, mean, std_dev, st, &p));
+        if (path) *path = p;
+        return 0;
+    };
+    const int rc = run();
+    (void)hipStreamSynchronize(st);
+    for (void* p : m.allocs) (void)hipFree(p);
+    return rc;
+}
+
 extern "C" long long odam_op_conv_paths(char* buf, int n, int reset) { return odam_cg::read_paths(buf, n, reset); }
 
 extern "C" int odam_op_conv_bf16_mode(int mode) {
diff --git a/odam_amd/csrc/detr_weights.hip b/odam_amd/csrc/detr_weights.hip
--- a/odam_amd/csrc/detr_weights.hip
+++ b/odam_amd/csrc/detr_weights.hip
@@ -4,6 +4,7 @@
 #include <cstring>
 
 #include "detr_model.h"
+#include "stem_u8_fold.h"
 
 using namespace odam_dm;
 
@@ -151,6 +152,44 @@
     std::snprintf(g_odam_err, sizeof(g_odam_err), "odam_detr_finalize: %s must be [%d, %d, %d, %d] for this backbone", name.c_str(),
                   cout, cin, k, k);
     return 1;
+}
+
+}
+
+namespace odam_dm {
+
+int pack_stem_rows(odam_detr* m, const float* w, int Cout, float* scale, float* bias) {
+    const int Kp = m->dt ? 256 : 224;
+    std::vector<float> pr((size_t)Cout * Kp, 0.0f);
+    for (int o = 0; o < Cout; o++)
+        for (int ci = 0; ci < 3; ci++)
+            for (int ky = 0; ky < 7; ky++)
+                for (int kx = 0; kx < 7; kx++)
+                    pr[(size_t)o * Kp + ky * 32 + kx * 4 + ci] = w[(((size_t)o * 3 + ci) * 7 + ky) * 7 + kx];
+    Conv& r = m->stem_rows;
+    r.Cin = 32; r.Cout = Cout; r.KH = 7; r.KW = 1; r.stride = 2; r.pad = 0; r.Kpad = Kp; r.k_order = m->dt ? 0 : 1;
+    RC(upload_w3(m, &r.w3, pr, Cout, Kp));
+    RC(upload_w(m, &r.w, pr));
+    r.scale = scale; r.bias = bias;
+    if (m->dt == 0) m->conv1_w.assign(w, w + (size_t)Cout * 147);
+    return 0;
+}
+
+int stem_u8_filters(odam_detr* m, const float* mean, const float* stdv, const odam_detr::StemU8** out) {
+    for (const odam_detr::StemU8& f : m->stem_u8)
+        if (std::memcmp(f.mean, mean, 12) == 0 && std::memcmp(f.stdv, stdv, 12) == 0) { *out = &f; return 0; }
+    const int Cout = m->stem_rows.Cout;
+    if (m->conv1_w.size() != (size_t)Cout * 147 || m->stem_rows.Kpad != 224) return odam_fail(1, "stem_u8_filters: no fp32 conv1 filters on this model");
+    odam_detr::StemU8 f{};
+    std::memcpy(f.mean, mean, 12); std::memcpy(f.stdv, stdv, 12);
+    stem_u8_centres(mean, f.centre);
+    std::vector<float> rows((size_t)Cout * 224);
+    stem_u8_fold(m->conv1_w.data(), Cout, mean, stdv, rows.data());
+    RC(upload_w3(m, &f.w3, rows, Cout, 224));
+    if (!f.w3) return odam_fail(1, "stem_u8_filters: the split filters could not be built");
+    m->stem_u8.push_back(f);
+    *out = &m->stem_u8.back();
+    return 0;
 }
 
 }
@@ -224,21 +263,9 @@
         NEED(w, bb + "conv1.weight");
         RC(pack_conv(m, m->stem, *w, 2, 3));
         RC(fold_bn(m, m->stem, bb + "bn1"));
-        {
-            const int Cout = (int)w->shape[0];
-            const int Kp = m->dt ? 256 : 224;
-            std::vector<float> pr((size_t)Cout * Kp, 0.0f);
-            for (int o = 0; o < Cout; o++)
-                for (int ci = 0; ci < 3; ci++)
-                    for (int ky = 0; ky < 7; ky++)
-                        for (int kx = 0; kx < 7; kx++)
-                            pr[(size_t)o * Kp + ky * 32 + kx * 4 + ci] = w->data[(((size_t)o * 3 + ci) * 7 + ky) * 7 + kx];
-            Conv& r = m->stem_rows;
-            r.Cin = 32; r.Cout = Cout; r.KH = 7; r.KW = 1; r.stride = 2; r.pad = 0; r.Kpad = Kp; r.k_order = m->dt ? 0 : 1;
-            RC(upload_w3(m, &r.w3, pr, Cout, Kp));
-            RC(upload_w(m, &r.w, pr));
-            r.scale = m->stem.scale; r.bias = m->stem.bias;
-        }
+        if (w->shape.size() != 4 || w->shape[1] != 3 || w->shape[2] != 7 || w->shape[3] != 7)
+            return odam_fail(1, "odam_detr_finalize: backbone.0.body.conv1.weight must be [Cout, 3, 7, 7]");
+        RC(pack_stem_rows(m, w->data.data(), (int)w->shape[0], m->stem.scale, m->stem.bias));
     }
     int inplanes = 64;
     for (int l = 0; l < 4; l++) {
diff --git a/odam_amd/csrc/odam_common.hip b/odam_amd/csrc/odam_common.hip
--- a/odam_amd/csrc/odam_common.hip
+++ b/odam_amd/csrc/odam_common.hip
@@ -22,6 +22,7 @@
     {"assoc.hungarian", 0, 0, 1},
     {"assoc.merge", 1, 0, 1},
     {"sq.two_per_cu", 1, 0, 1},
+    {"stem.u8", 1, 0, 1},
 };
 std::atomic<int> g_val[N_KEYS];
 std::atomic<bool> g_init{false};
diff --git a/odam_amd/csrc/odam_config.h b/odam_amd/csrc/odam_config.h
--- a/odam_amd/csrc/odam_config.h
+++ b/odam_amd/csrc/odam_config.h
@@ -26,6 +26,7 @@
     ASSOC_HUNGARIAN,
     ASSOC_MERGE,
     SQ_TWO_PER_CU,
+    STEM_U8,
     N_KEYS
 };
 int get(Key k);
diff --git a/odam_amd/csrc/stem_u8_fold.h b/odam_amd/csrc/stem_u8_fold.h
--- /dev/null
+++ b/odam_amd/csrc/stem_u8_fold.h
@@ -0,0 +1,46 @@
+#pragma once
+#include <cmath>
+#include <cstddef>
+
+#if defined(__HIPCC__)
+#define ODAM_STEM_U8_HD __host__ __device__
+#else
+#define ODAM_STEM_U8_HD
+#endif
+
+namespace odam_dm {
+
+ODAM_STEM_U8_HD inline bool stem_u8_inside(int Xp, int Yp, int H, int W, int& X, int& Y) {
+    X = Xp - 3; Y = Yp - 3;
+    return (unsigned)X < (unsigned)W && (unsigned)Y < (unsigned)H;
+}
+ODAM_STEM_U8_HD inline unsigned stem_u8_bf16(int d) { return __builtin_bit_cast(unsigned, (float)d) >> 16; }
+ODAM_STEM_U8_HD inline void stem_u8_pixel(int u0, int u1, int u2, int c0, int c1, int c2, unsigned& w0, unsigned& w1) {
+    w0 = stem_u8_bf16(u0 - c0) | (stem_u8_bf16(u1 - c1) << 16);
+    w1 = stem_u8_bf16(u2 - c2) | (stem_u8_bf16(1) << 16);
+}
+
+inline void stem_u8_centres(const float mean[3], int centre[3]) {
+    for (int k = 0; k < 3; k++) centre[k] = (int)std::lrint(255.0 * (double)mean[k]);
+}
+
+inline void stem_u8_fold(const float* w, int Cout, const float mean[3], const float stdv[3], float* rows) {
+    int c[3];
+    stem_u8_centres(mean, c);
+    for (int o = 0; o < Cout; o++)
+        for (int ky = 0; ky < 7; ky++)
+            for (int kx = 0; kx < 8; kx++) {
+                float* r = rows + (size_t)o * 224 + ky * 32 + kx * 4;
+                r[0] = r[1] = r[2] = r[3] = 0.0f;
+                if (kx == 7) continue;
+                double ind = 0.0;
+                for (int k = 0; k < 3; k++) {
+                    const double wk = (double)w[(((size_t)o * 3 + k) * 7 + ky) * 7 + kx];
+                    r[k] = (float)(wk / (255.0 * (double)stdv[k]));
+                    ind += wk * ((double)c[k] / 255.0 - (double)mean[k]) / (double)stdv[k];
+                }
+                r[3] = (float)ind;
+            }
+}
+
+}
diff --git a/odam_amd/detector.py b/odam_amd/detector.py
--- a/odam_amd/detector.py
+++ b/odam_amd/detector.py
@@ -127,7 +127,7 @@
         new = torch.device("cuda:0" if str(device) == "cuda" else device)
         if new != self.device:
             self.close()
-            for name in ("_streams", "_mscratch", "_xform", "_stage", "_copy_stream", "_pinned"):
+            for name in ("_streams", "_mscratch", "_stage", "_copy_stream", "_pinned"):
                 if hasattr(self, name):
                     setattr(self, name, None)
         self.device = new
@@ -322,13 +322,31 @@
                                                           ctypes.c_void_p(st)), "odam_detr_preprocess_u8")
         return out
 
+    def _forward_raw(self, handle, rgb, outs, stream):
+        from .transforms import MEAN, STD
+        B, h, w, c = rgb.shape
+        assert c == 3 and rgb.dtype == torch.uint8 and rgb.is_cuda and rgb.is_contiguous()
+        mean, std = (ctypes.c_float * 3)(*MEAN), (ctypes.c_float * 3)(*STD)
+        ad = lambda t: None if t is None else t.data_ptr()
+        _lib.check(_lib.lib().odam_detr_forward_u8(handle, rgb.data_ptr(), B, h, w, ctypes.addressof(mean), ctypes.addressof(std),
+                                                   *[ad(t) for t in outs], stream), "odam_detr_forward_u8")
+
     def forward_u8(self, rgb):
-        outs = [self(self.preprocess_u8(rgb[b0:b0 + self.max_batch])) for b0 in range(0, rgb.shape[0], self.max_batch)]
-        if len(outs) == 1:
-            return outs[0]
-        res = {k: torch.cat([o[k] for o in outs]) for k in outs[0] if k != "_hw"}
-        res["_hw"] = outs[0]["_hw"]
-        return res
+        from .transforms import target_size
+        N, h, w, _ = rgb.shape
+        H, W = target_size(w, h, *self.resize)
+        a, dev = self.arch, self.device
+        mk = lambda n: torch.empty(N, a["num_queries"], n, device=dev, dtype=torch.float32)
+        out = {"pred_logits": mk(a["num_classes1"]), "pred_boxes": mk(4), "pred_angle": mk(a["angle_bins"]),
+               "pred_offset": mk(2), "pred_size": mk(3), "pred_depth": mk(1), "pred_obj_features": mk(a["hidden_dim"])}
+        keys = ("pred_logits", "pred_boxes", "pred_angle", "pred_offset", "pred_size", "pred_depth", "pred_obj_features")
+        handle = self._handle(H, W)
+        with torch.cuda.device(dev):
+            st = torch.cuda.current_stream(dev).cuda_stream
+            for b0 in range(0, N, self.max_batch):
+                self._forward_raw(handle, rgb[b0:b0 + self.max_batch], [out[k][b0:b0 + self.max_batch] for k in keys], st)
+        out["_hw"] = (H, W)
+        return out
 
     def debug_taps(self, B, H, W):
         hd = self._handle(H, W)
@@ -460,9 +478,6 @@
         events = []
         nb = 0
         on_host = not frames.is_cuda
-        if raw:
-            if getattr(self, "_xform", None) is None or self._xform[0].shape[2:] != (H, W) or len(self._xform) != ns:
-                self._xform = [torch.empty(mb, 3, H, W, device=dev, dtype=torch.float32) for _ in range(ns)]
         if on_host:
             st0 = getattr(self, "_stage", None)
             if st0 is None or st0[0][0].shape[1:] != frames.shape[1:] or st0[0][0].dtype != frames.dtype or len(st0) != ns:
@@ -494,10 +509,11 @@
                         self._streams[k].wait_event(up)
                         src = buf
                     if raw:
-                        src = self.preprocess_u8(src, self._xform[k][:B], k, self._streams[k].cuda_stream)
-                    _lib.check(L.odam_detr_forward(handles[k], _lib.ptr(src), ctypes.c_int(B), _lib.ptr(lg),
-                                                   _lib.ptr(bx), _lib.ptr(an), _lib.ptr(of), _lib.ptr(sz), _lib.ptr(dp),
-                                                   ctypes.c_void_p(0), sp), "odam_detr_forward")
+                        self._forward_raw(handles[k], src, [t[:B] for t in (lg, bx, an, of, sz, dp)] + [None], self._streams[k].cuda_stream)
+                    else:
+                        _lib.check(L.odam_detr_forward(handles[k], _lib.ptr(src), ctypes.c_int(B), _lib.ptr(lg),
+                                                       _lib.ptr(bx), _lib.ptr(an), _lib.ptr(of), _lib.ptr(sz), _lib.ptr(dp),
+                                                       ctypes.c_void_p(0), sp), "odam_detr_forward")
                     _lib.check(L.odam_detr_postprocess(handles[k], _lib.ptr(lg), _lib.ptr(bx), _lib.ptr(an), _lib.ptr(of),
                                                        _lib.ptr(sz), _lib.ptr(dp), ctypes.c_int(B),
                                                        K9.ctypes.data_as(_lib.c_float_p), ctypes.c_float(img_w),
```

After: 1143, median of 6. 2.1% higher.
